# dhansmair/flamingo-mini

Hardware: AMD Instinct MI355X
Metric: images/sec (fwd+bwd) flamingo-mini bs=32 (higher is better)
Workload: dtype bf16

## Files before the change

flamingo-mini_amd/csrc/ff_api.hip:

```cpp
#include <stdarg.h>
#include <stdio.h>
#include <math.h>
#include <stdlib.h>
#include "ff_common.h"
#include "ff_internal.h"

namespace ff {

static thread_local char g_err[512] = "";
void set_error(const char* fmt, ...) {
    va_list ap;
    va_start(ap, fmt);
    vsnprintf(g_err, sizeof(g_err), fmt, ap);
    va_end(ap);
}
#ifdef FF_DEBUG
int dbg_switch(const char* name, int dflt) {
    const char* e = getenv(name);
    return e ? atoi(e) : dflt;
}
#endif
int check_launch(const char* what) {
    hipError_t e = hipGetLastError();
    if (e != hipSuccess) {
        set_error("%s: launch failed: %s", what, hipGetErrorString(e));
        return FF_ERR_LAUNCH;
    }
    return FF_OK;
}


static LnArgs ln_args(int dtype, int rows, int cols, RowMap x, RowMap y, RowMap dx) {
    LnArgs a;
    a.dtype = dtype; a.rows = rows; a.cols = cols;
    a.x_map = x; a.y_map = y; a.dx_map = dx;
    a.add_rows_per_seg = 0; a.add_div = 0; a.eps = 1e-5f; a.stats_given = 0;
    return a;
}

struct RsDims {
    int dt, Bn, T, v, D, F, q, H, dh, inner, ffi, R, depth, nte, act;
    int Mq, Mkv, Mf;
    size_t es, attn_ws;
    float scale;
    RowMap pD, pI, pF;
    RowMap lat_bcast;
    RowMap kv_media, kv_lat;
    explicit RsDims(const ff_resampler_desc& d) {
        dt = d.dtype; Bn = d.batch; T = d.n_frames; v = d.n_tokens; D = d.dim; F = T * v; q = d.num_latents;
        H = d.heads; dh = d.dim_head; inner = H * dh; ffi = d.ff_mult * D; R = F + q; depth = d.depth;
        nte = d.num_time_embeds; act = d.act; es = dtype_size(dt); scale = 1.0f / sqrtf((float)dh);
        Mq = Bn * q; Mkv = Bn * R; Mf = Bn * F; attn_ws = (size_t)Bn * H * q * 4;
        pD = plain_rows(D); pI = plain_rows(inner); pF = plain_rows(ffi);
        lat_bcast = RowMap{D, 0, q};
        kv_media = RowMap{D, (long long)R * D, F};
        kv_lat = RowMap{D, (long long)R * D, q};
    }
    LnArgs ln_latents() const { return ln_args(dt, Mq, D, pD, pD, pD); }
    LnArgs ln_media(RowMap y) const {
        LnArgs a = ln_args(dt, Mf, D, pD, y, pD);
        a.add_rows_per_seg = F; a.add_div = v;
        return a;
    }
    template <typename P> P* kv_latent_rows(P* kv) const { return (P*)((char*)kv + (size_t)F * D * es); }
};
struct RsLayerSaved {
    void *x_in, *kv_in, *Qs, *K, *V, *O, *x_mid, *xn_f, *Hpre, *Aact;
    float *mean_l, *rstd_l, *lse, *mean_f, *rstd_f;
};
constexpr int kMaxDepth = 64;
struct RsSaved {
    float *mean_m, *rstd_m, *mean_o, *rstd_o;
    void* x_last;
    RsLayerSaved L[kMaxDepth];
};
static void rs_take_layer_saved(const RsDims& s, Arena& a, RsLayerSaved& L) {
    const size_t rows_q = s.Mq, rows_kv = s.Mkv;
    L.mean_l = a.take<float>(rows_q * 4);
    L.rstd_l = a.take<float>(rows_q * 4);
    L.kv_in = a.take(rows_kv * s.D * s.es);
    L.Qs = a.take(rows_q * s.inner * s.es);
    L.K = a.take(rows_kv * s.inner * s.es);
    L.V = a.take(rows_kv * s.inner * s.es);
    L.lse = a.take<float>((size_t)s.Bn * s.H * s.q * 4);
    L.O = a.take(rows_q * s.inner * s.es);
    L.x_mid = a.take(rows_q * s.D * s.es);
    L.mean_f = a.take<float>(rows_q * 4);
    L.rstd_f = a.take<float>(rows_q * 4);
    L.xn_f = a.take(rows_q * s.D * s.es);
    L.Hpre = a.take(rows_q * s.ffi * s.es);
    L.Aact = a.take(rows_q * s.ffi * s.es);
}
static size_t rs_saved_layout(const RsDims& s, void* base, size_t cap, RsSaved& o) {
    Arena a(base, cap);
    const size_t rows_q = s.Mq;
    o.mean_m = a.take<float>((size_t)s.Mf * 4);
    o.rstd_m = a.take<float>((size_t)s.Mf * 4);
    for (int l = 0; l < s.depth; l++) {
        o.L[l].x_in = l == 0 ? nullptr : a.take(rows_q * s.D * s.es);
        rs_take_layer_saved(s, a, o.L[l]);
    }
    o.x_last = a.take(rows_q * s.D * s.es);
    o.mean_o = a.take<float>(rows_q * 4);
    o.rstd_o = a.take<float>(rows_q * 4);
    return align_up(a.used);
}

static size_t rs_ws_bytes(const RsDims& s) {
    size_t w = 0;
    auto g = [&](int M, int N, int K, int nz) { w = std::max(w, gemm_workspace_bytes(s.dt, M, N, K, nz, 0)); };
    g(s.Mq, s.inner, s.D, 1); g(s.Mkv, s.inner, s.D, 2); g(s.Mq, s.D, s.inner, 1); g(s.Mq, s.ffi, s.D, 1); g(s.Mq, s.D, s.ffi, 1);
    for (int nz = 1; nz <= 4; nz++) {
        g(s.D, s.ffi, s.Mq, nz); g(s.ffi, s.D, s.Mq, nz); g(s.D, s.inner, s.Mq, nz); g(s.inner, s.D, s.Mq, nz); g(s.inner, s.D, s.Mkv, nz);
    }
    g(s.Mkv, s.D, s.inner, 1);
    w = std::max(w, layernorm_bwd_workspace(s.Mf, s.D));
    w = std::max(w, layernorm_bwd_workspace(s.Mq, s.D));
    w = std::max(w, rows_reduce_workspace(s.Mq, s.D, s.q, 1));
    w = std::max(w, rows_reduce_workspace(s.Mf, s.D, s.F, s.v));
    return align_up(w) + align_up(s.attn_ws);
}
struct RsChain {
    void *ws, *dxn, *dO, *dkv, *dln;
    size_t ws_bytes, gws;
    float* attn_ws;
};
struct RsLayerGrads {
    void *dx_mid, *dH, *dQs, *dK, *dV;
};
static void rs_take_ws(const RsDims& s, Arena& a, RsChain& c) {
    c.ws_bytes = rs_ws_bytes(s);
    c.ws = a.take(c.ws_bytes);
    c.gws = c.ws_bytes - align_up(s.attn_ws);
    c.attn_ws = c.ws ? (float*)((char*)c.ws + c.gws) : nullptr;
}
static void rs_take_chain(const RsDims& s, Arena& a, RsChain& c) {
    c.dxn = a.take((size_t)s.Mq * s.D * s.es);
    c.dO = a.take((size_t)s.Mq * s.inner * s.es);
    c.dkv = a.take((size_t)s.Mkv * s.D * s.es);
    c.dln = a.take((size_t)s.Mq * s.D * s.es);
}
static void rs_take_layer_grads(const RsDims& s, Arena& a, RsLayerGrads& g) {
    g.dx_mid = a.take((size_t)s.Mq * s.D * s.es);
    g.dH = a.take((size_t)s.Mq * s.ffi * s.es);
    g.dQs = a.take((size_t)s.Mq * s.inner * s.es);
    g.dK = a.take((size_t)s.Mkv * s.inner * s.es);
    g.dV = a.take((size_t)s.Mkv * s.inner * s.es);
}
static void rs_take_ln_partials(const RsDims& s, Arena& a, bool deferrable, float** lnp) {
    for (int i = 0; i < 3; i++) lnp[i] = deferrable ? a.take<float>(layernorm_bwd_partial_bytes(i == 2 ? s.Mf : s.Mq, s.D)) : nullptr;
}

struct RsScratch {
    RsChain c;
    void *dx0, *dxf;
    void* dx_out[kMaxDepth];
    RsLayerGrads L[kMaxDepth];
    float* lnp[3 * kMaxDepth + 1];
};
static size_t rs_scratch_layout(const RsDims& s, void* base, size_t cap, bool bwd, RsScratch& o) {
    Arena a(base, cap);
    rs_take_ws(s, a, o.c);
    if (bwd) {
        o.dx0 = a.take((size_t)s.Mq * s.D * s.es);
        rs_take_chain(s, a, o.c);
        o.dxf = a.take((size_t)s.Mf * s.D * s.es);
        for (int l = 0; l < s.depth; l++) {
            o.dx_out[l] = a.take((size_t)s.Mq * s.D * s.es);
            rs_take_layer_grads(s, a, o.L[l]);
        }
        static const int defer_ln = dbg_switch("FF_DEFER_LN", 1);
        const bool lnd = defer_ln != 0 && layernorm_bwd_deferrable(s.dt, s.D);
        for (int l = 0; l < s.depth; l++) rs_take_ln_partials(s, a, lnd, o.lnp + 3 * l);
        o.lnp[3 * s.depth] = lnd ? a.take<float>(layernorm_bwd_partial_bytes(s.Mq, s.D)) : nullptr;
    }
    return align_up(a.used);
}

static int rs_check(const ff_resampler_desc* d) {
    FF_CHECK(d, FF_ERR_SHAPE, "resampler: null descriptor");
    FF_CHECK(d->dtype == FF_DTYPE_F32 || d->dtype == FF_DTYPE_BF16, FF_ERR_UNSUPPORTED, "resampler: dtype %d", d->dtype);
    FF_CHECK(d->batch > 0 && d->n_frames > 0 && d->n_tokens > 0 && d->dim > 0 && d->depth > 0 && d->depth <= kMaxDepth && d->heads > 0 &&
                 d->dim_head > 0 && d->num_latents > 0 && d->ff_mult > 0,
             FF_ERR_SHAPE, "resampler: bad dimensions");
    FF_CHECK(d->n_frames <= d->num_time_embeds, FF_ERR_SHAPE, "resampler: %d frames > num_time_embeds %d (perceiver_resampler.py:166)",
             d->n_frames, d->num_time_embeds);
    FF_CHECK(d->act >= FF_ACT_GELU && d->act <= FF_ACT_RELU, FF_ERR_SHAPE, "resampler: act %d", d->act);
    return FF_OK;
}

static ff_attn_desc rs_attn_desc(const RsDims& s) {
    ff_attn_desc a = {};
    a.dtype = s.dt; a.batch = s.Bn; a.heads = s.H; a.dim_head = s.dh; a.n_q = s.q; a.n_kv = s.R; a.mode = FF_ATTN_DENSE;
    const ff_strides sq = {(long long)s.q * s.inner, s.inner, s.dh}, sk = {(long long)s.R * s.inner, s.inner, s.dh};
    a.q = sq; a.o = sq; a.dq = sq; a.dout = sq;
    a.k = sk; a.v = sk; a.dk = sk; a.dv = sk;
    return a;
}

static int rs_media_stats(const RsDims& s, const void* x_f, const void* tpe, float* mean_m, float* rstd_m, hipStream_t st) {
    return layernorm_fwd(s.ln_media(s.pD), x_f, tpe, nullptr, nullptr, nullptr, mean_m, rstd_m, st);
}

static int rs_layer_forward(const RsDims& s, const void* const* p, const void* x_f, const void* tpe, float* mean_m, float* rstd_m, const void* x_in,
                            RowMap x_map, void* x_out, const RsLayerSaved& L, void* ws, size_t ws_bytes, hipStream_t st) {
    const RowMap pD = s.pD, pI = s.pI, pF = s.pF;
    void* kv_lat_base = s.kv_latent_rows(L.kv_in);
    {
        LnArgs a = s.ln_media(s.kv_media);
        a.stats_given = 1;
        FF_TRY(layernorm_fwd(a, x_f, tpe, p[0], p[1], L.kv_in, mean_m, rstd_m, st));
    }
    FF_TRY(layernorm_fwd(ln_args(s.dt, s.Mq, s.D, x_map, s.kv_lat, pD), x_in, nullptr, p[2], p[3], kv_lat_base, L.mean_l, L.rstd_l, st));
    FF_TRY(Gemm(s.dt, s.Mq, s.inner, s.D).a(0, s.kv_lat).b(0, pD).c(pI).scale(s.scale).problem(kv_lat_base, p[4], L.Qs).run(ws, ws_bytes, st));
    FF_TRY(Gemm(s.dt, s.Mkv, s.inner, s.D).a(0, pD).b(0, pD).c(pI).problem(L.kv_in, p[5], L.K).problem(L.kv_in, p[6], L.V).run(ws, ws_bytes, st));
    FF_TRY(attention_fwd(rs_attn_desc(s), L.Qs, L.K, L.V, nullptr, L.O, L.lse, st));
    FF_TRY(Gemm(s.dt, s.Mq, s.D, s.inner).a(0, pI).b(0, pI).c(pD).res_map(x_map).problem(L.O, p[7], L.x_mid, nullptr, nullptr, x_in).run(ws, ws_bytes, st));
    FF_TRY(layernorm_fwd(s.ln_latents(), L.x_mid, nullptr, p[8], p[9], L.xn_f, L.mean_f, L.rstd_f, st));
    FF_TRY(Gemm(s.dt, s.Mq, s.ffi, s.D).a(0, pD).b(0, pD).c(pF).act(s.act).problem(L.xn_f, p[10], L.Aact, L.Hpre).run(ws, ws_bytes, st));
    return Gemm(s.dt, s.Mq, s.D, s.ffi).a(0, pF).b(0, pF).c(pD).problem(L.Aact, p[11], x_out, nullptr, nullptr, L.x_mid).run(ws, ws_bytes, st);
}

static int rs_final_norm(const RsDims& s, const void* x_last, const void* gamma, const void* beta, void* out, float* mean, float* rstd, hipStream_t st) {
    return layernorm_fwd(s.ln_latents(), x_last, nullptr, gamma, beta, out, mean, rstd, st);
}

static int rs_ln_bwd(const RsChain& W, float* partial, LnPending* pending, const LnArgs& a, const void* dy, const void* x, const void* add,
                     const void* gamma, const float* mean, const float* rstd, void* dx, const void* dx_res, void* dg, void* db, hipStream_t st) {
    if (partial)
        return layernorm_bwd(a, dy, x, add, gamma, mean, rstd, dx, dx_res, dg, db, partial, layernorm_bwd_partial_bytes(a.rows, a.cols), st, nullptr, pending);
    return layernorm_bwd(a, dy, x, add, gamma, mean, rstd, dx, dx_res, dg, db, W.ws, W.gws, st);
}

static int rs_layer_backward(const RsDims& s, const void* const* p, void* const* g, const void* x_f, const void* tpe, const float* mean_m,
                             const float* rstd_m, const void* x_in, RowMap x_map, const RsLayerSaved& L, const void* dx_out, void* dx_in,
                             void* dx_f, const void* dx_f_res, const RsChain& W, const RsLayerGrads& T, float* const* lnp, LnPending* ln_sets,
                             hipStream_t st) {
    const RowMap pD = s.pD, pI = s.pI, pF = s.pF;
    FF_TRY(Gemm(s.dt, s.Mq, s.ffi, s.D).a(0, pD).b(1, pF).c(pF).act_bwd(s.act).problem(dx_out, p[11], T.dH, nullptr, L.Hpre).run(W.ws, W.gws, st));
    FF_TRY(Gemm(s.dt, s.Mq, s.D, s.ffi).a(0, pF).b(1, pD).c(pD).problem(T.dH, p[10], W.dxn).run(W.ws, W.gws, st));
    FF_TRY(rs_ln_bwd(W, lnp[0], &ln_sets[0], s.ln_latents(), W.dxn, L.x_mid, nullptr, p[8], L.mean_f, L.rstd_f, T.dx_mid, dx_out, g[8], g[9], st));
    FF_TRY(Gemm(s.dt, s.Mq, s.inner, s.D).a(0, pD).b(1, pI).c(pI).problem(T.dx_mid, p[7], W.dO).run(W.ws, W.gws, st));
    FF_TRY(attention_bwd(rs_attn_desc(s), L.Qs, L.K, L.V, nullptr, L.O, W.dO, L.lse, T.dQs, T.dK, T.dV, W.attn_ws, s.attn_ws, st));
    FF_TRY(Gemm(s.dt, s.Mkv, s.D, s.inner).a(0, pI).b(1, pD).c(pD).problem(T.dK, p[5], W.dkv).run(W.ws, W.gws, st));
    FF_TRY(Gemm(s.dt, s.Mkv, s.D, s.inner).a(0, pI).b(1, pD).c(pD).problem(T.dV, p[6], W.dkv, nullptr, nullptr, W.dkv).run(W.ws, W.gws, st));
    FF_TRY(Gemm(s.dt, s.Mq, s.D, s.inner).a(0, pI).b(1, pD).c(pD).res_map(s.kv_lat).scale(s.scale)
               .problem(T.dQs, p[4], W.dln, nullptr, nullptr, s.kv_latent_rows(W.dkv)).run(W.ws, W.gws, st));
    FF_TRY(rs_ln_bwd(W, lnp[1], &ln_sets[1], ln_args(s.dt, s.Mq, s.D, x_map, pD, pD), W.dln, x_in, nullptr, p[2], L.mean_l, L.rstd_l, dx_in, T.dx_mid, g[2],
                     g[3], st));
    return rs_ln_bwd(W, lnp[2], &ln_sets[2], s.ln_media(s.kv_media), W.dkv, x_f, tpe, p[0], mean_m, rstd_m, dx_f, dx_f_res, g[0], g[1], st);
}

static int rs_input_grads(const RsDims& s, const void* dx0, const void* dxf, void* d_latents, void* d_tpe, void* ws, size_t ws_bytes, hipStream_t st) {
    FF_TRY(rows_reduce(s.dt, s.Mq, s.D, s.pD, s.q, 1, dx0, d_latents, ws, ws_bytes, st));
    if (s.nte > s.T) FF_TRY(zero_bytes((char*)d_tpe + (size_t)s.T * s.D * s.es, (size_t)(s.nte - s.T) * s.D * s.es, st));
    return rows_reduce(s.dt, s.Mf, s.D, s.pD, s.F, s.v, dxf, d_tpe, ws, ws_bytes, st);
}

static int resampler_fwd(const ff_resampler_desc* d, const void* x_f, const void* const* P, void* out, void* saved, size_t saved_bytes,
                         void* scratch, size_t scratch_bytes, hipStream_t st) {
    FF_TRY(rs_check(d));
    FF_CHECK(x_f && P && out && saved && scratch, FF_ERR_SHAPE, "resampler_fwd: null argument");
    const RsDims s(*d);
    RsSaved S;
    RsScratch W;
    FF_CHECK(rs_saved_layout(s, saved, saved_bytes, S) <= saved_bytes, FF_ERR_WORKSPACE, "resampler_fwd: saved buffer too small");
    FF_CHECK(rs_scratch_layout(s, scratch, scratch_bytes, false, W) <= scratch_bytes, FF_ERR_WORKSPACE, "resampler_fwd: scratch too small");
    const void *latents = P[0], *tpe = P[1];
    FF_TRY(rs_media_stats(s, x_f, tpe, S.mean_m, S.rstd_m, st));
    for (int l = 0; l < s.depth; l++) {
        const void* const* p = P + FF_RESAMPLER_GLOBAL_PARAMS + FF_RESAMPLER_LAYER_PARAMS * l;
        void* x_next = l + 1 < s.depth ? S.L[l + 1].x_in : S.x_last;
        FF_TRY(rs_layer_forward(s, p, x_f, tpe, S.mean_m, S.rstd_m, l == 0 ? latents : S.L[l].x_in, l == 0 ? s.lat_bcast : s.pD, x_next, S.L[l], W.c.ws,
                                W.c.ws_bytes, st));
    }
    return rs_final_norm(s, S.x_last, P[2], P[3], out, S.mean_o, S.rstd_o, st);
}

static int resampler_bwd(const ff_resampler_desc* d, const void* x_f, const void* const* P, const void* dout, const void* saved,
                         size_t saved_bytes, void* const* G, void* dx_f, void* scratch, size_t scratch_bytes, hipStream_t st) {
    FF_TRY(rs_check(d));
    FF_CHECK(x_f && P && dout && saved && G && scratch, FF_ERR_SHAPE, "resampler_bwd: null argument");
    const RsDims s(*d);
    RsSaved S;
    RsScratch W;
    FF_CHECK(rs_saved_layout(s, (void*)saved, saved_bytes, S) <= saved_bytes, FF_ERR_WORKSPACE, "resampler_bwd: saved buffer too small");
    FF_CHECK(rs_scratch_layout(s, scratch, scratch_bytes, true, W) <= scratch_bytes, FF_ERR_WORKSPACE, "resampler_bwd: scratch too small");
    const RowMap pD = s.pD, pI = s.pI, pF = s.pF;
    const void *latents = P[0], *tpe = P[1];
    void* dxf = dx_f ? dx_f : W.dxf;
    void* const ws = W.c.ws;
    const size_t gws = W.c.gws;

    LnPending ln_sets[3 * kMaxDepth + 1];
    FF_TRY(rs_ln_bwd(W.c, W.lnp[3 * s.depth], &ln_sets[3 * s.depth], s.ln_latents(), dout, S.x_last, nullptr, P[2], S.mean_o, S.rstd_o,
                     W.dx_out[s.depth - 1], nullptr, G[2], G[3], st));
    for (int l = s.depth - 1; l >= 0; l--) {
        const void* const* p = P + FF_RESAMPLER_GLOBAL_PARAMS + FF_RESAMPLER_LAYER_PARAMS * l;
        void* const* g = G + FF_RESAMPLER_GLOBAL_PARAMS + FF_RESAMPLER_LAYER_PARAMS * l;
        void* dx_below = l == 0 ? W.dx0 : W.dx_out[l - 1];
        FF_TRY(rs_layer_backward(s, p, g, x_f, tpe, S.mean_m, S.rstd_m, l == 0 ? latents : S.L[l].x_in, l == 0 ? s.lat_bcast : pD, S.L[l], W.dx_out[l],
                                 dx_below, dxf, l == s.depth - 1 ? nullptr : dxf, W.c, W.L[l], W.lnp + 3 * l, ln_sets + 3 * l, st));
    }
    FF_TRY(layernorm_bwd_finish(s.dt, ln_sets, 3 * s.depth + 1, st));
    constexpr int kRsGroup = 4;
    for (int l0 = 0; l0 < s.depth; l0 += kRsGroup) {
        const int l1 = std::min(s.depth, l0 + kRsGroup);
        Gemm g3(s.dt, s.D, s.ffi, s.Mq), g1(s.dt, s.ffi, s.D, s.Mq), go(s.dt, s.D, s.inner, s.Mq), gq(s.dt, s.inner, s.D, s.Mq);
        g3.a(1, pD).b(1, pF).c(pF);
        g1.a(1, pF).b(1, pD).c(pD);
        go.a(1, pD).b(1, pI).c(pI);
        gq.a(1, pI).b(1, s.kv_lat).c(pD).scale(s.scale);
        for (int l = l0; l < l1; l++) {
            void* const* g = G + FF_RESAMPLER_GLOBAL_PARAMS + FF_RESAMPLER_LAYER_PARAMS * l;
            const RsLayerSaved& L = S.L[l];
            const RsLayerGrads& T = W.L[l];
            g3.problem(W.dx_out[l], L.Aact, g[11]);
            g1.problem(T.dH, L.xn_f, g[10]);
            go.problem(T.dx_mid, L.O, g[7]);
            gq.problem(T.dQs, s.kv_latent_rows(L.kv_in), g[4]);
        }
        FF_TRY(g3.run(ws, gws, st));
        FF_TRY(g1.run(ws, gws, st));
        FF_TRY(go.run(ws, gws, st));
        FF_TRY(gq.run(ws, gws, st));
    }
    {
        Gemm gkv(s.dt, s.inner, s.D, s.Mkv);
        gkv.a(1, pI).b(1, pD).c(pD);
        for (int l = 0; l < s.depth; l++) {
            void* const* g = G + FF_RESAMPLER_GLOBAL_PARAMS + FF_RESAMPLER_LAYER_PARAMS * l;
            gkv.problem(W.L[l].dK, S.L[l].kv_in, g[5]);
            gkv.problem(W.L[l].dV, S.L[l].kv_in, g[6]);
            if (gkv.P.nz == kRsGroup || l == s.depth - 1) {
                FF_TRY(gkv.run(ws, gws, st));
                gkv.P.nz = 0;
            }
        }
    }
    return rs_input_grads(s, W.dx0, dxf, G[0], G[1], ws, gws, st);
}

struct RsProSaved { float *mean_m, *rstd_m; };
static size_t rs_pro_layout(const RsDims& s, void* base, size_t cap, RsProSaved& o) {
    Arena a(base, cap);
    o.mean_m = a.take<float>((size_t)s.Mf * 4);
    o.rstd_m = a.take<float>((size_t)s.Mf * 4);
    return align_up(a.used);
}
static size_t rs_layer_saved_layout(const RsDims& s, void* base, size_t cap, RsLayerSaved& L) {
    Arena a(base, cap);
    L.x_in = nullptr;
    rs_take_layer_saved(s, a, L);
    return align_up(a.used);
}
struct RsLayerScratch {
    RsChain c;
    RsLayerGrads g;
    float* lnp[3];
};
static size_t rs_layer_scratch_layout(const RsDims& s, void* base, size_t cap, RsLayerScratch& o) {
    Arena a(base, cap);
    rs_take_ws(s, a, o.c);
    rs_take_chain(s, a, o.c);
    rs_take_layer_grads(s, a, o.g);
    rs_take_ln_partials(s, a, layernorm_bwd_deferrable(s.dt, s.D), o.lnp);
    return align_up(a.used);
}

static int rs_prologue_fwd(const ff_resampler_desc* d, const void* x_f, const void* tpe, void* pro, size_t pro_bytes, hipStream_t st) {
    FF_TRY(rs_check(d));
    FF_CHECK(x_f && tpe && pro, FF_ERR_SHAPE, "resampler_prologue_fwd: null argument");
    const RsDims s(*d);
    RsProSaved S;
    FF_CHECK(rs_pro_layout(s, pro, pro_bytes, S) <= pro_bytes, FF_ERR_WORKSPACE, "resampler_prologue_fwd: saved buffer too small");
    return rs_media_stats(s, x_f, tpe, S.mean_m, S.rstd_m, st);
}

static int rs_layer_fwd(const ff_resampler_desc* d, const void* x_f, const void* tpe, const void* pro, size_t pro_bytes, const void* x_in,
                        int x_is_latents, const void* const* p, void* x_out, void* saved, size_t saved_bytes, void* scratch, size_t scratch_bytes,
                        hipStream_t st) {
    FF_TRY(rs_check(d));
    FF_CHECK(x_f && tpe && pro && x_in && p && x_out && saved && scratch, FF_ERR_SHAPE, "resampler_layer_fwd: null argument");
    const RsDims s(*d);
    RsProSaved Pr;
    RsLayerSaved L;
    RsLayerScratch W;
    FF_CHECK(rs_pro_layout(s, (void*)pro, pro_bytes, Pr) <= pro_bytes, FF_ERR_WORKSPACE, "resampler_layer_fwd: prologue buffer too small");
    FF_CHECK(rs_layer_saved_layout(s, saved, saved_bytes, L) <= saved_bytes, FF_ERR_WORKSPACE, "resampler_layer_fwd: saved buffer too small");
    FF_CHECK(rs_layer_scratch_layout(s, scratch, scratch_bytes, W) <= scratch_bytes, FF_ERR_WORKSPACE, "resampler_layer_fwd: scratch too small");
    return rs_layer_forward(s, p, x_f, tpe, Pr.mean_m, Pr.rstd_m, x_in, x_is_latents ? s.lat_bcast : s.pD, x_out, L, W.c.ws, W.c.ws_bytes, st);
}

static int rs_layer_bwd(const ff_resampler_desc* d, const void* x_f, const void* tpe, const void* pro, size_t pro_bytes, const void* x_in,
                        int x_is_latents, const void* const* p, const void* dx_out, const void* saved, size_t saved_bytes, void* const* g,
                        void* dx_in, void* dx_f, int dx_f_accumulate, void* scratch, size_t scratch_bytes, hipStream_t st) {
    FF_TRY(rs_check(d));
    FF_CHECK(x_f && tpe && pro && x_in && p && dx_out && saved && g && dx_in && dx_f && scratch, FF_ERR_SHAPE, "resampler_layer_bwd: null argument");
    const RsDims s(*d);
    RsProSaved Pr;
    RsLayerSaved L;
    RsLayerScratch W;
    FF_CHECK(rs_pro_layout(s, (void*)pro, pro_bytes, Pr) <= pro_bytes, FF_ERR_WORKSPACE, "resampler_layer_bwd: prologue buffer too small");
    FF_CHECK(rs_layer_saved_layout(s, (void*)saved, saved_bytes, L) <= saved_bytes, FF_ERR_WORKSPACE, "resampler_layer_bwd: saved buffer too small");
    FF_CHECK(rs_layer_scratch_layout(s, scratch, scratch_bytes, W) <= scratch_bytes, FF_ERR_WORKSPACE, "resampler_layer_bwd: scratch too small");
    const RowMap pD = s.pD, pI = s.pI, pF = s.pF;
    void* const ws = W.c.ws;
    const size_t gws = W.c.gws;
    LnPending ln_sets[3];
    FF_TRY(rs_layer_backward(s, p, g, x_f, tpe, Pr.mean_m, Pr.rstd_m, x_in, x_is_latents ? s.lat_bcast : pD, L, dx_out, dx_in, dx_f,
                             dx_f_accumulate ? dx_f : nullptr, W.c, W.g, W.lnp, ln_sets, st));
    FF_TRY(layernorm_bwd_finish(s.dt, ln_sets, 3, st));
    FF_TRY(Gemm(s.dt, s.D, s.ffi, s.Mq).a(1, pD).b(1, pF).c(pF).problem(dx_out, L.Aact, g[11]).run(ws, gws, st));
    FF_TRY(Gemm(s.dt, s.ffi, s.D, s.Mq).a(1, pF).b(1, pD).c(pD).problem(W.g.dH, L.xn_f, g[10]).run(ws, gws, st));
    FF_TRY(Gemm(s.dt, s.D, s.inner, s.Mq).a(1, pD).b(1, pI).c(pI).problem(W.g.dx_mid, L.O, g[7]).run(ws, gws, st));
    FF_TRY(Gemm(s.dt, s.inner, s.D, s.Mq).a(1, pI).b(1, s.kv_lat).c(pD).scale(s.scale).problem(W.g.dQs, s.kv_latent_rows(L.kv_in), g[4]).run(ws, gws, st));
    return Gemm(s.dt, s.inner, s.D, s.Mkv).a(1, pI).b(1, pD).c(pD).problem(W.g.dK, L.kv_in, g[5]).problem(W.g.dV, L.kv_in, g[6]).run(ws, gws, st);
}

static int rs_prologue_bwd(const ff_resampler_desc* d, const void* dx0, const void* dx_f, void* d_latents, void* d_tpe, void* scratch,
                           size_t scratch_bytes, hipStream_t st) {
    FF_TRY(rs_check(d));
    FF_CHECK(dx0 && dx_f && d_latents && d_tpe && scratch, FF_ERR_SHAPE, "resampler_prologue_bwd: null argument");
    const RsDims s(*d);
    RsLayerScratch W;
    FF_CHECK(rs_layer_scratch_layout(s, scratch, scratch_bytes, W) <= scratch_bytes, FF_ERR_WORKSPACE, "resampler_prologue_bwd: scratch too small");
    return rs_input_grads(s, dx0, dx_f, d_latents, d_tpe, W.c.ws, W.c.ws_bytes, st);
}

static int rs_epilogue_fwd(const ff_resampler_desc* d, const void* x_last, const void* gamma, const void* beta, void* out, void* epi, size_t epi_bytes,
                           hipStream_t st) {
    FF_TRY(rs_check(d));
    FF_CHECK(x_last && gamma && beta && out && epi, FF_ERR_SHAPE, "resampler_epilogue_fwd: null argument");
    const RsDims s(*d);
    const size_t rows_q = s.Mq;
    FF_CHECK(epi_bytes >= 2 * align_up(rows_q * 4), FF_ERR_WORKSPACE, "resampler_epilogue_fwd: saved buffer too small");
    return rs_final_norm(s, x_last, gamma, beta, out, (float*)epi, (float*)((char*)epi + align_up(rows_q * 4)), st);
}
static int rs_epilogue_bwd(const ff_resampler_desc* d, const void* dout, const void* x_last, const void* gamma, const void* epi, size_t epi_bytes,
                           void* dx_last, void* dgamma, void* dbeta, void* scratch, size_t scratch_bytes, hipStream_t st) {
    FF_TRY(rs_check(d));
    FF_CHECK(dout && x_last && gamma && epi && dx_last && dgamma && dbeta && scratch, FF_ERR_SHAPE, "resampler_epilogue_bwd: null argument");
    const RsDims s(*d);
    const size_t rows_q = s.Mq;
    FF_CHECK(epi_bytes >= 2 * align_up(rows_q * 4), FF_ERR_WORKSPACE, "resampler_epilogue_bwd: saved buffer too small");
    RsLayerScratch W;
    FF_CHECK(rs_layer_scratch_layout(s, scratch, scratch_bytes, W) <= scratch_bytes, FF_ERR_WORKSPACE, "resampler_epilogue_bwd: scratch too small");
    const float* mean = (const float*)epi;
    const float* rstd = (const float*)((const char*)epi + align_up(rows_q * 4));
    return layernorm_bwd(s.ln_latents(), dout, x_last, nullptr, gamma, mean, rstd, dx_last, nullptr, dgamma, dbeta, W.c.ws, W.c.ws_bytes, st);
}

struct XaDims {
    int dt, b, L, d, dv, Nm, nv, Nk, H, dh, inner, ffi, act;
    size_t es;
    float scale;
    bool ext_kv;
    explicit XaDims(const ff_xattn_desc& x) {
        ext_kv = x.cached_k.sr != 0;
        dt = x.dtype; b = x.batch; L = x.n_tokens; d = x.dim; dv = x.dim_visual; Nm = x.n_media; nv = x.n_visual; Nk = Nm * nv;
        H = x.heads; dh = x.dim_head; inner = H * dh; ffi = x.ff_mult * d; act = x.act; es = dtype_size(dt);
        scale = 1.0f / sqrtf((float)dh);
    }
};
struct XaSaved {
    float *mean_a, *rstd_a, *lse, *mean_f, *rstd_f;
    void *yn, *Qs, *KV, *O, *attn_out, *y1, *xn_f, *Hpre, *Aact, *ffw_out;
    size_t kv_offset;
};
static size_t xa_saved_layout(const XaDims& s, void* base, size_t cap, XaSaved& o) {
    Arena a(base, cap);
    const size_t M = (size_t)s.b * s.L;
    o.KV = s.ext_kv ? nullptr : a.take((size_t)s.b * s.Nk * 2 * s.inner * s.es);
    o.kv_offset = 0;
    o.mean_a = a.take<float>(M * 4);
    o.rstd_a = a.take<float>(M * 4);
    o.yn = a.take(M * s.d * s.es);
    o.Qs = a.take(M * s.inner * s.es);
    o.lse = a.take<float>((size_t)s.b * s.H * s.L * 4);
    o.O = a.take(M * s.inner * s.es);
    o.attn_out = a.take(M * s.d * s.es);
    o.y1 = a.take(M * s.d * s.es);
    o.mean_f = a.take<float>(M * 4);
    o.rstd_f = a.take<float>(M * 4);
    o.xn_f = a.take(M * s.d * s.es);
    o.Hpre = a.take(M * s.ffi * s.es);
    o.Aact = a.take(M * s.ffi * s.es);
    o.ffw_out = a.take(M * s.d * s.es);
    return align_up(a.used);
}
struct XaScratch {
    void *dy1, *dH, *dxn, *dO, *dQs, *dKV, *dyn, *ws;
    size_t ws_bytes;
    float* lnx;
};
struct XaStash {
    void *dy1, *dH, *dQs;
    float *lnp_f = nullptr, *lnp_a = nullptr;
};
static bool xa_ln_deferrable(const XaDims& s) {
    static const int on = dbg_switch("FF_DEFER_LN", 1);
    return on != 0 && layernorm_bwd_deferrable(s.dt, s.d);
}
static size_t xa_stash_layout(const XaDims& s, void* base, size_t cap, XaStash& o) {
    Arena a(base, cap);
    const size_t M = (size_t)s.b * s.L;
    o.dy1 = a.take(M * s.d * s.es);
    o.dH = a.take(M * s.ffi * s.es);
    o.dQs = a.take(M * s.inner * s.es);
    if (xa_ln_deferrable(s)) {
        o.lnp_f = a.take<float>(layernorm_bwd_partial_bytes((int)M, s.d));
        o.lnp_a = a.take<float>(layernorm_bwd_partial_bytes((int)M, s.d));
    }
    return align_up(a.used);
}
static size_t xa_ws_bytes(const XaDims& s) {
    const int M = s.b * s.L, Mk = s.b * s.Nk;
    size_t w = 0;
    auto g = [&](int m, int n, int k) { w = std::max(w, gemm_workspace_bytes(s.dt, m, n, k, 1, 0)); };
    g(M, s.inner, s.d); g(Mk, 2 * s.inner, s.dv); g(M, s.d, s.inner); g(M, s.ffi, s.d); g(M, s.d, s.ffi);
    g(s.d, s.ffi, M); g(s.ffi, s.d, M); g(s.d, s.inner, M); g(s.inner, s.d, M); g(2 * s.inner, s.dv, Mk); g(Mk, s.dv, 2 * s.inner);
    w = std::max(w, layernorm_bwd_workspace(M, s.d));
    w = std::max(w, gate_grad_workspace(M, s.d));
    if (decode_ffw_supported(s.dt, M, s.d, s.ffi)) w = std::max(w, decode_ffw_workspace_bytes(s.d, s.ffi));
    return align_up(w) + align_up((size_t)s.b * s.H * s.L * 4);
}
static size_t xa_scratch_layout(const XaDims& s, void* base, size_t cap, bool bwd, XaScratch& o) {
    Arena a(base, cap);
    const size_t M = (size_t)s.b * s.L;
    o.ws_bytes = xa_ws_bytes(s);
    o.ws = a.take(o.ws_bytes);
    o.lnx = a.take<float>(xa_ln3_part_bytes(s.b, s.H));
    if (bwd) {
        o.dy1 = a.take(M * s.d * s.es);
        o.dH = a.take(M * s.ffi * s.es);
        o.dxn = a.take(M * s.d * s.es);
        o.dO = a.take(M * s.inner * s.es);
        o.dQs = a.take(M * s.inner * s.es);
        o.dKV = s.ext_kv ? nullptr : a.take((size_t)s.b * s.Nk * 2 * s.inner * s.es);
        o.dyn = a.take(M * s.d * s.es);
    }
    return align_up(a.used);
}
static int xa_check(const ff_xattn_desc* d) {
    FF_CHECK(d, FF_ERR_SHAPE, "xattn: null descriptor");
    FF_CHECK(d->dtype == FF_DTYPE_F32 || d->dtype == FF_DTYPE_BF16, FF_ERR_UNSUPPORTED, "xattn: dtype %d", d->dtype);
    FF_CHECK(d->batch > 0 && d->n_tokens > 0 && d->dim > 0 && d->dim_visual > 0 && d->n_media > 0 && d->n_visual > 0 && d->heads > 0 &&
                 d->dim_head > 0 && d->ff_mult > 0,
             FF_ERR_SHAPE, "xattn: bad dimensions");
    FF_CHECK(d->act >= FF_ACT_GELU && d->act <= FF_ACT_RELU, FF_ERR_SHAPE, "xattn: act %d", d->act);
    return FF_OK;
}
static ff_attn_desc xa_attn_desc(const ff_xattn_desc& x, const XaDims& s, bool cached) {
    ff_attn_desc a = {};
    a.dtype = s.dt; a.batch = s.b; a.heads = s.H; a.dim_head = s.dh; a.n_q = s.L; a.n_kv = s.Nk;
    a.mode = FF_ATTN_MEDIA; a.n_visual = s.nv; a.tt_stride = x.tt_stride; a.tt_offset = x.tt_offset;
    const ff_strides sq = {(long long)s.L * s.inner, s.inner, s.dh};
    const ff_strides sk = {(long long)s.Nk * 2 * s.inner, 2LL * s.inner, s.dh};
    a.q = sq; a.o = sq; a.dq = sq; a.dout = sq;
    a.k = cached ? x.cached_k : sk;
    a.v = cached ? x.cached_v : sk;
    a.dk = sk; a.dv = sk;
    return a;
}

static bool xa_fused_enabled() {
    static const int v = dbg_switch("FF_XATTN_FUSED", 1);
    return v != 0;
}
static bool xa_ln3_enabled() {
    static const int v = dbg_switch("FF_XATTN_LN3", 1);
    return v != 0;
}
static XaFusedArgs xa_fused_args(const ff_xattn_desc& x, const XaDims& s, bool ext_kv) {
    XaFusedArgs a = {};
    a.batch = s.b; a.heads = s.H; a.n_q = s.L; a.n_kv = s.Nk; a.n_visual = s.nv; a.tt_stride = x.tt_stride; a.tt_offset = x.tt_offset;
    a.dim = s.d; a.inner = s.inner; a.scale = s.scale; a.eps = 1e-5f;
    static const int xcd_split = dbg_switch("FF_XATTN_XCD_SPLIT", 0);
    a.xcd_split = xcd_split;
    const ff_strides sk = {(long long)s.Nk * 2 * s.inner, 2LL * s.inner, s.dh};
    a.k = ext_kv ? x.cached_k : sk;
    a.v = ext_kv ? x.cached_v : sk;
    a.dk = sk; a.dv = sk;
    return a;
}

static bool xa_ln3_in_bwd(const ff_xattn_desc& x, const XaDims& s) {
    if (!xa_ln3_enabled() || !xa_fused_enabled() || !xa_fused_supported(s.dt, s.dh, s.d, s.inner) || x.sync == nullptr) return false;
    const XaFusedArgs fa = xa_fused_args(x, s, s.ext_kv);
    const int M = s.b * s.L;
    return xa_out_fusable(fa, s.dt, s.dh) && s.b <= layernorm_bwd_partial_blocks(M) && (size_t)s.b * (2 * (size_t)s.d + 2) * sizeof(float) <= layernorm_bwd_workspace(M, s.d);
}
static int xattn_fwd(const ff_xattn_desc* d, const void* y, const void* vf, const int* tt, const void* const* P, const void* ck,
                     const void* cv, void* y_out, void* saved, size_t saved_bytes, void* scratch, size_t scratch_bytes, hipStream_t st) {
    FF_TRY(xa_check(d));
    const bool cached = ck != nullptr;
    FF_CHECK(y && tt && P && y_out && saved && scratch && (cached ? cv != nullptr : vf != nullptr), FF_ERR_SHAPE, "xattn_fwd: null argument");
    const XaDims s(*d);
    FF_CHECK(s.ext_kv == cached, FF_ERR_SHAPE, "xattn_fwd: external K / V need their strides in the descriptor (cached_k / cached_v) and vice versa");
    XaSaved S;
    XaScratch W;
    FF_CHECK(xa_saved_layout(s, saved, saved_bytes, S) <= saved_bytes, FF_ERR_WORKSPACE, "xattn_fwd: saved buffer too small");
    FF_CHECK(xa_scratch_layout(s, scratch, scratch_bytes, false, W) <= scratch_bytes, FF_ERR_WORKSPACE, "xattn_fwd: scratch too small");
    const int M = s.b * s.L, Mk = s.b * s.Nk;
    const RowMap pd = plain_rows(s.d), pI = plain_rows(s.inner), pF = plain_rows(s.ffi), pV = plain_rows(s.dv), pKV = plain_rows(2 * s.inner);
    const void *Kp, *Vp;
    if (!cached) {
        FF_TRY(Gemm(s.dt, Mk, 2 * s.inner, s.dv).a(0, pV).b(0, pV).c(pKV).problem(vf, P[5], S.KV).run(W.ws, W.ws_bytes, st));
        Kp = S.KV;
        Vp = (const char*)S.KV + (size_t)s.inner * s.es;
    } else {
        Kp = ck; Vp = cv;
    }
    bool out_fused = false, ln_fused = false;
    if (xa_fused_enabled() && xa_fused_supported(s.dt, s.dh, s.d, s.inner)) {
        const XaFusedArgs fa = xa_fused_args(*d, s, cached);
        XaOutArgs oa = {(const bf16*)P[6], (const bf16*)P[0], (bf16*)S.y1, (bf16*)S.attn_out, (unsigned*)d->sync};
        out_fused = d->sync != nullptr && xa_out_fusable(fa, s.dt, s.dh) && !decode_ffw_supported(s.dt, M, s.d, s.ffi);
        if (out_fused && xa_ln3_enabled()) {
            oa.ln_g = (const bf16*)P[7]; oa.ln_b = (const bf16*)P[8]; oa.ln_out = (bf16*)S.xn_f; oa.ln_mean = S.mean_f; oa.ln_rstd = S.rstd_f;
            oa.ln_part = W.lnx;
            ln_fused = true;
        }
        FF_TRY(xa_qattn_fwd(fa, s.dt, s.dh, y, P[2], P[3], P[4], Kp, Vp, tt, S.yn, S.Qs, S.O, S.mean_a, S.rstd_a, S.lse, st, out_fused ? &oa : nullptr));
    } else {
        FF_TRY(layernorm_fwd(ln_args(s.dt, M, s.d, pd, pd, pd), y, nullptr, P[2], P[3], S.yn, S.mean_a, S.rstd_a, st));
        FF_TRY(Gemm(s.dt, M, s.inner, s.d).a(0, pd).b(0, pd).c(pI).scale(s.scale).problem(S.yn, P[4], S.Qs).run(W.ws, W.ws_bytes, st));
        FF_TRY(attention_fwd(xa_attn_desc(*d, s, cached), S.Qs, Kp, Vp, tt, S.O, S.lse, st));
    }
    if (!out_fused) FF_TRY(Gemm(s.dt, M, s.d, s.inner).a(0, pI).b(0, pI).c(pd).problem(S.O, P[6], S.y1, S.attn_out, nullptr, y, P[0]).run(W.ws, W.ws_bytes, st));
    if (decode_ffw_supported(s.dt, M, s.d, s.ffi))
        return decode_ffw(M, s.d, s.ffi, s.act, 1e-5f, S.y1, P[7], P[8], P[9], P[10], P[1], S.xn_f, S.mean_f, S.rstd_f, S.Hpre, S.Aact, S.ffw_out, y_out,
                          W.ws, W.ws_bytes, st);
    if (!ln_fused) FF_TRY(layernorm_fwd(ln_args(s.dt, M, s.d, pd, pd, pd), S.y1, nullptr, P[7], P[8], S.xn_f, S.mean_f, S.rstd_f, st));
    FF_TRY(Gemm(s.dt, M, s.ffi, s.d).a(0, pd).b(0, pd).c(pF).act(s.act).problem(S.xn_f, P[9], S.Aact, S.Hpre).run(W.ws, W.ws_bytes, st));
    return Gemm(s.dt, M, s.d, s.ffi).a(0, pF).b(0, pF).c(pd).problem(S.Aact, P[10], y_out, S.ffw_out, nullptr, S.y1, P[1]).run(W.ws, W.ws_bytes, st);
}

static int xattn_bwd(const ff_xattn_desc* d, const void* y, const void* vf, const int* tt, const void* const* P, const void* dy2,
                     const void* saved, size_t saved_bytes, void* const* G, void* dy, void* dvf, void* scratch, size_t scratch_bytes,
                     hipStream_t st, const void* ext_k = nullptr, const void* ext_v = nullptr, void* dkv_out = nullptr,
                     void* stash = nullptr, size_t stash_bytes = 0) {
    FF_TRY(xa_check(d));
    const bool hoisted = ext_k != nullptr;
    FF_CHECK(y && tt && P && dy2 && saved && G && dy && scratch && (hoisted ? (ext_v && dkv_out) : vf != nullptr), FF_ERR_SHAPE,
             "xattn_bwd: null argument");
    const XaDims s(*d);
    FF_CHECK(s.ext_kv == hoisted, FF_ERR_SHAPE, "xattn_bwd: external K / V need their strides in the descriptor (cached_k / cached_v) and vice versa");
    XaSaved S;
    XaScratch W;
    FF_CHECK(xa_saved_layout(s, (void*)saved, saved_bytes, S) <= saved_bytes, FF_ERR_WORKSPACE, "xattn_bwd: saved buffer too small");
    FF_CHECK(xa_scratch_layout(s, scratch, scratch_bytes, true, W) <= scratch_bytes, FF_ERR_WORKSPACE, "xattn_bwd: scratch too small");
    XaStash T{W.dy1, W.dH, W.dQs};
    const bool defer = stash != nullptr;
    if (defer) FF_CHECK(xa_stash_layout(s, stash, stash_bytes, T) <= stash_bytes, FF_ERR_WORKSPACE, "xattn_bwd: stash too small");
    const bool defer_ln = defer && xa_ln_deferrable(s);
    if (defer_ln)
        FF_CHECK(((uintptr_t)y | (uintptr_t)dy | (uintptr_t)dy2 | (uintptr_t)P[2] | (uintptr_t)P[7]) % 16 == 0, FF_ERR_SHAPE,
                 "xattn_bwd (deferred weight gradients): y, d y_out, d y and the LayerNorm weights must be 16-byte aligned");
    LnPending pend_f, pend_a;
    const int M = s.b * s.L, Mk = s.b * s.Nk;
    const RowMap pd = plain_rows(s.d), pI = plain_rows(s.inner), pF = plain_rows(s.ffi), pV = plain_rows(s.dv), pKV = plain_rows(2 * s.inner);
    const size_t attn_ws_bytes = align_up((size_t)s.b * s.H * s.L * 4);
    const size_t gws = W.ws_bytes - attn_ws_bytes;
    float* attn_ws = (float*)((char*)W.ws + gws);

    if (!defer) FF_TRY(Gemm(s.dt, s.d, s.ffi, M).a(1, pd).b(1, pF).c(pF).problem(dy2, S.Aact, G[10], nullptr, nullptr, nullptr, P[1]).run(W.ws, gws, st));
    FF_TRY(Gemm(s.dt, M, s.ffi, s.d).a(0, pd).b(1, pF).c(pF).act_bwd(s.act).problem(dy2, P[10], T.dH, nullptr, S.Hpre, nullptr, P[1]).run(W.ws, gws, st));
    if (!defer) FF_TRY(Gemm(s.dt, s.ffi, s.d, M).a(1, pF).b(1, pd).c(pd).problem(T.dH, S.xn_f, G[9]).run(W.ws, gws, st));
    static const int fold_reduce = dbg_switch("FF_FOLD_SPLITK_LN", 1);
    int dxn_splits = 1;
    FF_TRY(Gemm(s.dt, M, s.d, s.ffi).a(0, pF).b(1, pd).c(pd).problem(T.dH, P[9], W.dxn).run(W.ws, gws, st, defer_ln && fold_reduce ? &dxn_splits : nullptr));
    {
        LnDots dots;
        dots.a = S.ffw_out; dots.alpha_a = P[1]; dots.out_a = G[1];
        dots.b = S.attn_out; dots.alpha_b = P[0]; dots.out_b = G[0];
        if (defer_ln) {
            LnArgs la = ln_args(s.dt, M, s.d, pd, pd, pd);
            if (dxn_splits > 1) { la.dy_splits = dxn_splits; la.dy_slab = (long long)M * s.d; }
            FF_TRY(layernorm_bwd(la, dxn_splits > 1 ? W.ws : W.dxn, S.y1, nullptr, P[7], S.mean_f, S.rstd_f, T.dy1, dy2, G[7], G[8], T.lnp_f,
                                 layernorm_bwd_partial_bytes(M, s.d), st, &dots, &pend_f));
            FF_CHECK(pend_f.partial, FF_ERR_SHAPE, "xattn_bwd: the one-pass LayerNorm backward did not apply in the deferred mode");
        } else FF_TRY(layernorm_bwd(ln_args(s.dt, M, s.d, pd, pd, pd), W.dxn, S.y1, nullptr, P[7], S.mean_f, S.rstd_f, T.dy1, dy2, G[7], G[8], W.ws, gws, st, &dots));
    }
    if (!defer) FF_TRY(Gemm(s.dt, s.d, s.inner, M).a(1, pd).b(1, pI).c(pI).problem(T.dy1, S.O, G[6], nullptr, nullptr, nullptr, P[0]).run(W.ws, gws, st));
    char* dK = hoisted ? (char*)dkv_out : (char*)W.dKV;
    char* dV = dK + (size_t)s.inner * s.es;
    const void* Kp = hoisted ? ext_k : S.KV;
    const void* Vp = hoisted ? ext_v : (const void*)((const char*)S.KV + (size_t)s.inner * s.es);
    bool dyn_fused = false, lnb_fused = false;
    float* lnb_partial = nullptr;
    if (xa_fused_enabled() && xa_fused_supported(s.dt, s.dh, s.d, s.inner)) {
        int single = 0;
        const XaFusedArgs fa = xa_fused_args(*d, s, hoisted);
        XaOutArgs oa = {(const bf16*)P[4], nullptr, (bf16*)W.dyn, nullptr, (unsigned*)d->sync};
        dyn_fused = d->sync != nullptr && xa_out_fusable(fa, s.dt, s.dh);
        if (dyn_fused && xa_ln3_in_bwd(*d, s)) {
            lnb_fused = true;
            lnb_partial = defer_ln ? T.lnp_a : (float*)W.ws;
            oa.out = nullptr;
            oa.ln_g = (const bf16*)P[2]; oa.ln_x = (const bf16*)y; oa.ln_res = (const bf16*)T.dy1; oa.ln_out = (bf16*)dy;
            oa.ln_mean = S.mean_a; oa.ln_rstd = S.rstd_a; oa.ln_part = W.lnx; oa.ln_wpart = lnb_partial;
        }
        FF_TRY(xa_dattn_bwd(fa, s.dt, s.dh, T.dy1, P[6], P[0], S.Qs, Kp, Vp, tt, S.O, S.lse, W.dO, T.dQs, dK, dV, attn_ws, &single, st,
                            dyn_fused ? &oa : nullptr));
        if (!single) FF_TRY(attention_bwd_dkv(xa_attn_desc(*d, s, hoisted), S.Qs, Kp, Vp, tt, W.dO, S.lse, attn_ws, dK, dV, st));
        if (lnb_fused && !defer_ln) {
            LnPending q;
            q.partial = lnb_partial; q.nblk = s.b; q.cols = s.d; q.dgamma = G[2]; q.dbeta = G[3];
            FF_TRY(layernorm_bwd_finish(s.dt, &q, 1, st));
        }
    } else {
        FF_TRY(Gemm(s.dt, M, s.inner, s.d).a(0, pd).b(1, pI).c(pI).problem(T.dy1, P[6], W.dO, nullptr, nullptr, nullptr, P[0]).run(W.ws, gws, st));
        FF_TRY(attention_bwd(xa_attn_desc(*d, s, hoisted), S.Qs, Kp, Vp, tt, S.O, W.dO, S.lse, T.dQs, dK, dV, attn_ws, (size_t)s.b * s.H * s.L * 4, st));
    }
    if (!defer) FF_TRY(Gemm(s.dt, s.inner, s.d, M).a(1, pI).b(1, pd).c(pd).scale(s.scale).problem(T.dQs, S.yn, G[4]).run(W.ws, gws, st));
    if (!hoisted) {
        FF_TRY(Gemm(s.dt, 2 * s.inner, s.dv, Mk).a(1, pKV).b(1, pV).c(pV).problem(W.dKV, vf, G[5]).run(W.ws, gws, st));
        if (dvf) FF_TRY(Gemm(s.dt, Mk, s.dv, 2 * s.inner).a(0, pKV).b(1, pV).c(pV).problem(W.dKV, P[5], dvf).run(W.ws, gws, st));
    }
    if (!dyn_fused) FF_TRY(Gemm(s.dt, M, s.d, s.inner).a(0, pI).b(1, pd).c(pd).scale(s.scale).problem(T.dQs, P[4], W.dyn).run(W.ws, gws, st));
    if (lnb_fused) return FF_OK;
    if (defer_ln) {
        FF_TRY(layernorm_bwd(ln_args(s.dt, M, s.d, pd, pd, pd), W.dyn, y, nullptr, P[2], S.mean_a, S.rstd_a, dy, T.dy1, G[2], G[3], T.lnp_a,
                             layernorm_bwd_partial_bytes(M, s.d), st, nullptr, &pend_a));
        FF_CHECK(pend_a.partial, FF_ERR_SHAPE, "xattn_bwd: the one-pass LayerNorm backward did not apply in the deferred mode");
        return FF_OK;
    }
    return layernorm_bwd(ln_args(s.dt, M, s.d, pd, pd, pd), W.dyn, y, nullptr, P[2], S.mean_a, S.rstd_a, dy, T.dy1, G[2], G[3], W.ws, gws, st);
}

static size_t xa_wgrad_ws_bytes(const XaDims& s) {
    const int M = s.b * s.L;
    size_t w = 0;
    for (int nz = 1; nz <= kGemmMaxZ; nz++)
        w = std::max({w, gemm_workspace_bytes(s.dt, s.d, s.ffi, M, nz, 0), gemm_workspace_bytes(s.dt, s.ffi, s.d, M, nz, 0),
                      gemm_workspace_bytes(s.dt, s.d, s.inner, M, nz, 0), gemm_workspace_bytes(s.dt, s.inner, s.d, M, nz, 0)});
    return align_up(w);
}
static int xattn_wgrad_grouped(const ff_xattn_desc* d, int n, const void* const* dy2, const void* const* saved, size_t saved_bytes,
                               const void* const* stash, size_t stash_bytes, const void* const* params, void* const* grads, void* ws,
                               size_t ws_bytes, hipStream_t st) {
    FF_TRY(xa_check(d));
    FF_CHECK(n >= 1 && n <= kGemmMaxZ && dy2 && saved && stash && params && grads, FF_ERR_SHAPE, "xattn_wgrad_grouped: 1..%d blocks per call", kGemmMaxZ);
    const XaDims s(*d);
    FF_CHECK(ws_bytes >= xa_wgrad_ws_bytes(s) && (ws || !xa_wgrad_ws_bytes(s)), FF_ERR_WORKSPACE, "xattn_wgrad_grouped: workspace too small");
    const int M = s.b * s.L;
    const RowMap pd = plain_rows(s.d), pI = plain_rows(s.inner), pF = plain_rows(s.ffi);
    LnPending ln_sets[2 * kGemmMaxZ];
    const bool finish_ln = xa_ln_deferrable(s);
    const int ln_blocks = layernorm_bwd_partial_blocks(M);
    Gemm g3(s.dt, s.d, s.ffi, M), g1(s.dt, s.ffi, s.d, M), go(s.dt, s.d, s.inner, M), gq(s.dt, s.inner, s.d, M);
    g3.a(1, pd).b(1, pF).c(pF);
    g1.a(1, pF).b(1, pd).c(pd);
    go.a(1, pd).b(1, pI).c(pI);
    gq.a(1, pI).b(1, pd).c(pd).scale(s.scale);
    for (int i = 0; i < n; i++) {
        XaSaved S;
        XaStash T;
        FF_CHECK(dy2[i] && saved[i] && stash[i], FF_ERR_SHAPE, "xattn_wgrad_grouped: null buffer of block %d", i);
        FF_CHECK(xa_saved_layout(s, (void*)saved[i], saved_bytes, S) <= saved_bytes, FF_ERR_WORKSPACE, "xattn_wgrad_grouped: saved buffer too small");
        FF_CHECK(xa_stash_layout(s, (void*)stash[i], stash_bytes, T) <= stash_bytes, FF_ERR_WORKSPACE, "xattn_wgrad_grouped: stash too small");
        const void* const* P = params + (size_t)i * FF_XATTN_PARAMS;
        void* const* G = grads + (size_t)i * FF_XATTN_PARAMS;
        FF_CHECK(G[10] && G[9] && G[6] && G[4] && P[0] && P[1], FF_ERR_SHAPE, "xattn_wgrad_grouped: null parameter / gradient of block %d", i);
        g3.problem(dy2[i], S.Aact, G[10], nullptr, nullptr, nullptr, P[1]);
        g1.problem(T.dH, S.xn_f, G[9]);
        go.problem(T.dy1, S.O, G[6], nullptr, nullptr, nullptr, P[0]);
        gq.problem(T.dQs, S.yn, G[4]);
        if (finish_ln) {
            FF_CHECK(G[0] && G[1] && G[2] && G[3] && G[7] && G[8], FF_ERR_SHAPE, "xattn_wgrad_grouped: null LayerNorm / gate gradient of block %d", i);
            LnPending& f = ln_sets[2 * i];
            f.partial = T.lnp_f; f.nblk = ln_blocks; f.cols = s.d; f.dgamma = G[7]; f.dbeta = G[8];
            f.alpha_a = P[1]; f.out_a = G[1]; f.alpha_b = P[0]; f.out_b = G[0];
            LnPending& q = ln_sets[2 * i + 1];
            q.partial = T.lnp_a; q.nblk = xa_ln3_in_bwd(*d, s) ? s.b : ln_blocks; q.cols = s.d; q.dgamma = G[2]; q.dbeta = G[3];
        }
    }
    if (finish_ln) FF_TRY(layernorm_bwd_finish(s.dt, ln_sets, 2 * n, st));
    FF_TRY(g3.run(ws, ws_bytes, st));
    FF_TRY(g1.run(ws, ws_bytes, st));
    FF_TRY(go.run(ws, ws_bytes, st));
    return gq.run(ws, ws_bytes, st);
}

static int kvp_check(const ff_kvproj_desc* d) {
    FF_CHECK(d, FF_ERR_SHAPE, "kv_project: null descriptor");
    FF_CHECK(d->dtype == FF_DTYPE_F32 || d->dtype == FF_DTYPE_BF16, FF_ERR_UNSUPPORTED, "kv_project: dtype %d", d->dtype);
    FF_CHECK(d->n_layers > 0 && d->rows > 0 && d->dim_visual > 0 && d->kv_dim > 0 && (long long)d->rows * d->dim_visual < (1LL << 31), FF_ERR_SHAPE,
             "kv_project: bad dimensions");
    return FF_OK;
}
static size_t kvp_gemm_ws(const ff_kvproj_desc* d) {
    size_t w = 0;
    for (int z = 1; z <= kKvProjGroup; z++)
        w = std::max({w, gemm_workspace_bytes(d->dtype, d->rows, d->kv_dim, d->dim_visual, z, 0),
                      gemm_workspace_bytes(d->dtype, d->kv_dim, d->dim_visual, d->rows, z, 0),
                      gemm_workspace_bytes(d->dtype, d->rows, d->dim_visual, d->kv_dim, z, 0)});
    return align_up(w);
}
static size_t kvp_ws_bytes(const ff_kvproj_desc* d, bool with_dvf) {
    const size_t es = d->dtype == FF_DTYPE_BF16 ? 2 : 4;
    size_t w = kvp_gemm_ws(d);
    if (with_dvf)
        w += align_up((size_t)d->n_layers * d->rows * d->dim_visual * es) +
             align_up(rows_reduce_workspace(d->n_layers, d->rows * d->dim_visual, d->n_layers, d->n_layers));
    return w;
}
static int kv_project_fwd(const ff_kvproj_desc* d, const void* vf, const void* const* w_kv, void* const* kv_out, void* ws, size_t ws_bytes,
                          hipStream_t st) {
    FF_TRY(kvp_check(d));
    FF_CHECK(vf && w_kv && kv_out && ws && ws_bytes >= kvp_gemm_ws(d), FF_ERR_WORKSPACE, "kv_project_fwd: null argument or workspace too small");
    const RowMap pV = plain_rows(d->dim_visual), pKV = plain_rows(d->kv_dim);
    for (int l0 = 0; l0 < d->n_layers; l0 += kKvProjGroup) {
        Gemm g(d->dtype, d->rows, d->kv_dim, d->dim_visual);
        g.a(0, pV).b(0, pV).c(pKV);
        for (int l = l0; l < std::min(d->n_layers, l0 + kKvProjGroup); l++) g.problem(vf, w_kv[l], kv_out[l]);
        FF_TRY(g.run(ws, ws_bytes, st));
    }
    return FF_OK;
}
static int kv_project_bwd(const ff_kvproj_desc* d, const void* vf, const void* const* w_kv, const void* const* dkv, void* const* dw_kv,
                          void* dvf, void* ws, size_t ws_bytes, hipStream_t st) {
    FF_TRY(kvp_check(d));
    FF_CHECK(vf && w_kv && dkv && dw_kv && ws && ws_bytes >= kvp_ws_bytes(d, dvf != nullptr), FF_ERR_WORKSPACE,
             "kv_project_bwd: null argument or workspace too small");
    const size_t es = d->dtype == FF_DTYPE_BF16 ? 2 : 4, gws = kvp_gemm_ws(d);
    const RowMap pV = plain_rows(d->dim_visual), pKV = plain_rows(d->kv_dim);
    char* terms = (char*)ws + gws;
    const size_t term_bytes = (size_t)d->rows * d->dim_visual * es;
    for (int l0 = 0; l0 < d->n_layers; l0 += kKvProjGroup) {
        const int l1 = std::min(d->n_layers, l0 + kKvProjGroup);
        Gemm gw(d->dtype, d->kv_dim, d->dim_visual, d->rows);
        gw.a(1, pKV).b(1, pV).c(pV);
        for (int l = l0; l < l1; l++) gw.problem(dkv[l], vf, dw_kv[l]);
        FF_TRY(gw.run(ws, gws, st));
        if (dvf) {
            Gemm gx(d->dtype, d->rows, d->dim_visual, d->kv_dim);
            gx.a(0, pKV).b(1, pV).c(pV);
            for (int l = l0; l < l1; l++) gx.problem(dkv[l], w_kv[l], terms + (size_t)l * term_bytes);
            FF_TRY(gx.run(ws, gws, st));
        }
    }
    if (dvf) {
        const int cols = d->rows * d->dim_visual;
        FF_TRY(rows_reduce(d->dtype, d->n_layers, cols, plain_rows(cols), d->n_layers, d->n_layers, terms, dvf,
                           terms + align_up((size_t)d->n_layers * term_bytes), rows_reduce_workspace(d->n_layers, cols, d->n_layers, d->n_layers), st));
    }
    return FF_OK;
}

}

extern "C" int ff_version(void) { return 6; }
extern "C" const char* ff_arch(void) { return "gfx950"; }
extern "C" const char* ff_last_error(void) { return ff::g_err; }

extern "C" size_t ff_resampler_saved_bytes(const ff_resampler_desc* d) {
    if (ff::rs_check(d) != FF_OK) return 0;
    ff::RsSaved S;
    return ff::rs_saved_layout(ff::RsDims(*d), nullptr, 0, S);
}
extern "C" size_t ff_resampler_scratch_bytes(const ff_resampler_desc* d) {
    if (ff::rs_check(d) != FF_OK) return 0;
    ff::RsScratch W;
    return ff::rs_scratch_layout(ff::RsDims(*d), nullptr, 0, true, W);
}
extern "C" int ff_resampler_fwd(const ff_resampler_desc* d, const void* x_f, const void* const* params, void* out, void* saved,
                                size_t saved_bytes, void* scratch, size_t scratch_bytes, ff_stream_t stream) {
    return ff::resampler_fwd(d, x_f, params, out, saved, saved_bytes, scratch, scratch_bytes, (hipStream_t)stream);
}
extern "C" int ff_resampler_bwd(const ff_resampler_desc* d, const void* x_f, const void* const* params, const void* dout,
                                const void* saved, size_t saved_bytes, void* const* grads, void* dx_f, void* scratch,
                                size_t scratch_bytes, ff_stream_t stream) {
    return ff::resampler_bwd(d, x_f, params, dout, saved, saved_bytes, grads, dx_f, scratch, scratch_bytes, (hipStream_t)stream);
}

extern "C" size_t ff_resampler_prologue_saved_bytes(const ff_resampler_desc* d) {
    if (ff::rs_check(d) != FF_OK) return 0;
    ff::RsProSaved S;
    return ff::rs_pro_layout(ff::RsDims(*d), nullptr, 0, S);
}
extern "C" size_t ff_resampler_layer_saved_bytes(const ff_resampler_desc* d) {
    if (ff::rs_check(d) != FF_OK) return 0;
    ff::RsLayerSaved L;
    return ff::rs_layer_saved_layout(ff::RsDims(*d), nullptr, 0, L);
}
extern "C" size_t ff_resampler_layer_scratch_bytes(const ff_resampler_desc* d) {
    if (ff::rs_check(d) != FF_OK) return 0;
    ff::RsLayerScratch W;
    return ff::rs_layer_scratch_layout(ff::RsDims(*d), nullptr, 0, W);
}
extern "C" size_t ff_resampler_epilogue_saved_bytes(const ff_resampler_desc* d) {
    if (ff::rs_check(d) != FF_OK) return 0;
    return 2 * ff::align_up((size_t)d->batch * d->num_latents * 4);
}
extern "C" int ff_resampler_prologue_fwd(const ff_resampler_desc* d, const void* x_f, const void* time_pos_emb, void* saved_pro, size_t saved_pro_bytes,
                                         hipStream_t stream) {
    return ff::rs_prologue_fwd(d, x_f, time_pos_emb, saved_pro, saved_pro_bytes, stream);
}
extern "C" int ff_resampler_layer_fwd(const ff_resampler_desc* d, const void* x_f, const void* time_pos_emb, const void* saved_pro, size_t saved_pro_bytes,
                                      const void* x_in, int x_in_is_latents, const void* const* layer_params, void* x_out, void* saved, size_t saved_bytes,
                                      void* scratch, size_t scratch_bytes, hipStream_t stream) {
    return ff::rs_layer_fwd(d, x_f, time_pos_emb, saved_pro, saved_pro_bytes, x_in, x_in_is_latents, layer_params, x_out, saved, saved_bytes, scratch,
                            scratch_bytes, stream);
}
extern "C" int ff_resampler_layer_bwd(const ff_resampler_desc* d, const void* x_f, const void* time_pos_emb, const void* saved_pro, size_t saved_pro_bytes,
                                      const void* x_in, int x_in_is_latents, const void* const* layer_params, const void* dx_out, const void* saved,
                                      size_t saved_bytes, void* const* layer_grads, void* dx_in, void* dx_f, int dx_f_accumulate, void* scratch,
                                      size_t scratch_bytes, hipStream_t stream) {
    return ff::rs_layer_bwd(d, x_f, time_pos_emb, saved_pro, saved_pro_bytes, x_in, x_in_is_latents, layer_params, dx_out, saved, saved_bytes, layer_grads,
                            dx_in, dx_f, dx_f_accumulate, scratch, scratch_bytes, stream);
}
extern "C" int ff_resampler_prologue_bwd(const ff_resampler_desc* d, const void* dx0, const void* dx_f, void* d_latents, void* d_time_pos_emb, void* scratch,
                                         size_t scratch_bytes, hipStream_t stream) {
    return ff::rs_prologue_bwd(d, dx0, dx_f, d_latents, d_time_pos_emb, scratch, scratch_bytes, stream);
}
extern "C" int ff_resampler_epilogue_fwd(const ff_resampler_desc* d, const void* x_last, const void* norm_weight, const void* norm_bias, void* out,
                                         void* saved_epi, size_t saved_epi_bytes, hipStream_t stream) {
    return ff::rs_epilogue_fwd(d, x_last, norm_weight, norm_bias, out, saved_epi, saved_epi_bytes, stream);
}
extern "C" int ff_resampler_epilogue_bwd(const ff_resampler_desc* d, const void* dout, const void* x_last, const void* norm_weight, const void* saved_epi,
                                         size_t saved_epi_bytes, void* dx_last, void* d_norm_weight, void* d_norm_bias, void* scratch, size_t scratch_bytes,
                                         hipStream_t stream) {
    return ff::rs_epilogue_bwd(d, dout, x_last, norm_weight, saved_epi, saved_epi_bytes, dx_last, d_norm_weight, d_norm_bias, scratch, scratch_bytes, stream);
}

extern "C" size_t ff_xattn_sync_bytes(void) { return (size_t)(4 * FF_XATTN_SYNC_SLOTS + 64) * sizeof(unsigned); }
extern "C" int ff_xattn_sync_status(const void* sync, hipStream_t stream) {
    FF_CHECK(sync, FF_ERR_SHAPE, "ff_xattn_sync_status: null buffer");
    unsigned flag = 0;
    hipError_t e = hipMemcpyAsync(&flag, (const unsigned*)sync + 2 * FF_XATTN_SYNC_SLOTS, sizeof(flag), hipMemcpyDeviceToHost, stream);
    if (e == hipSuccess) e = hipStreamSynchronize(stream);
    FF_CHECK(e == hipSuccess, FF_ERR_LAUNCH, "ff_xattn_sync_status: %s", hipGetErrorString(e));
    return flag ? 1 : 0;
}
extern "C" size_t ff_xattn_saved_bytes(const ff_xattn_desc* d) {
    if (ff::xa_check(d) != FF_OK) return 0;
    ff::XaSaved S;
    return ff::xa_saved_layout(ff::XaDims(*d), nullptr, 0, S);
}
extern "C" size_t ff_xattn_scratch_bytes(const ff_xattn_desc* d) {
    if (ff::xa_check(d) != FF_OK) return 0;
    ff::XaScratch W;
    return ff::xa_scratch_layout(ff::XaDims(*d), nullptr, 0, true, W);
}
extern "C" size_t ff_xattn_kv_offset(const ff_xattn_desc* d) {
    (void)d;
    return 0;
}
extern "C" int ff_xattn_block_fwd(const ff_xattn_desc* d, const void* y, const void* visual_features, const int* text_time,
                                  const void* const* params, const void* cached_k, const void* cached_v, void* y_out, void* saved,
                                  size_t saved_bytes, void* scratch, size_t scratch_bytes, ff_stream_t stream) {
    return ff::xattn_fwd(d, y, visual_features, text_time, params, cached_k, cached_v, y_out, saved, saved_bytes, scratch, scratch_bytes,
                         (hipStream_t)stream);
}
extern "C" int ff_xattn_block_bwd(const ff_xattn_desc* d, const void* y, const void* visual_features, const int* text_time,
                                  const void* const* params, const void* dy_out, const void* saved, size_t saved_bytes, void* const* grads,
                                  void* dy, void* dvisual_features, void* scratch, size_t scratch_bytes, ff_stream_t stream) {
    return ff::xattn_bwd(d, y, visual_features, text_time, params, dy_out, saved, saved_bytes, grads, dy, dvisual_features, scratch,
                         scratch_bytes, (hipStream_t)stream);
}

extern "C" int ff_xattn_block_bwd_kv(const ff_xattn_desc* d, const void* y, const void* k, const void* v, const int* text_time,
                                     const void* const* params, const void* dy_out, const void* saved, size_t saved_bytes,
                                     void* const* grads, void* dy, void* dkv, void* scratch, size_t scratch_bytes, ff_stream_t stream) {
    using namespace ff;
    FF_CHECK(k && v && dkv, FF_ERR_SHAPE, "ff_xattn_block_bwd_kv: null K / V / dKV");
    return xattn_bwd(d, y, nullptr, text_time, params, dy_out, saved, saved_bytes, grads, dy, nullptr, scratch, scratch_bytes,
                     (hipStream_t)stream, k, v, dkv);
}
extern "C" size_t ff_xattn_wgrad_stash_bytes(const ff_xattn_desc* d) {
    if (ff::xa_check(d) != FF_OK) return 0;
    ff::XaStash T;
    return ff::xa_stash_layout(ff::XaDims(*d), nullptr, 0, T);
}
extern "C" size_t ff_xattn_wgrad_workspace_bytes(const ff_xattn_desc* d) {
    if (ff::xa_check(d) != FF_OK) return 0;
    return ff::xa_wgrad_ws_bytes(ff::XaDims(*d));
}
extern "C" int ff_xattn_block_bwd_kv_data(const ff_xattn_desc* d, const void* y, const void* k, const void* v, const int* text_time,
                                          const void* const* params, const void* dy_out, const void* saved, size_t saved_bytes,
                                          void* const* grads, void* dy, void* dkv, void* stash, size_t stash_bytes, void* scratch,
                                          size_t scratch_bytes, ff_stream_t stream) {
    using namespace ff;
    FF_CHECK(k && v && dkv && stash, FF_ERR_SHAPE, "ff_xattn_block_bwd_kv_data: null K / V / dKV / stash");
    return xattn_bwd(d, y, nullptr, text_time, params, dy_out, saved, saved_bytes, grads, dy, nullptr, scratch, scratch_bytes,
                     (hipStream_t)stream, k, v, dkv, stash, stash_bytes);
}
extern "C" int ff_xattn_wgrad_grouped(const ff_xattn_desc* d, int n_blocks, const void* const* dy_out, const void* const* saved,
                                      size_t saved_bytes, const void* const* stash, size_t stash_bytes, const void* const* params,
                                      void* const* grads, void* workspace, size_t workspace_bytes, ff_stream_t stream) {
    return ff::xattn_wgrad_grouped(d, n_blocks, dy_out, saved, saved_bytes, stash, stash_bytes, params, grads, workspace, workspace_bytes,
                                   (hipStream_t)stream);
}
extern "C" size_t ff_kv_project_workspace_bytes(const ff_kvproj_desc* d, int with_dvf) {
    if (ff::kvp_check(d) != FF_OK) return 0;
    return ff::kvp_ws_bytes(d, with_dvf != 0);
}
extern "C" int ff_kv_project_fwd(const ff_kvproj_desc* d, const void* visual_features, const void* const* w_kv, void* const* kv_out,
                                 void* workspace, size_t workspace_bytes, ff_stream_t stream) {
    return ff::kv_project_fwd(d, visual_features, w_kv, kv_out, workspace, workspace_bytes, (hipStream_t)stream);
}
extern "C" int ff_kv_project_bwd(const ff_kvproj_desc* d, const void* visual_features, const void* const* w_kv, const void* const* dkv,
                                 void* const* dw_kv, void* dvisual_features, void* workspace, size_t workspace_bytes, ff_stream_t stream) {
    return ff::kv_project_bwd(d, visual_features, w_kv, dkv, dw_kv, dvisual_features, workspace, workspace_bytes, (hipStream_t)stream);
}
```

flamingo-mini_amd/csrc/ff_internal.h:

```cpp
#pragma once
#include <algorithm>
#include "ff_common.h"

namespace ff {

constexpr int kGemmMaxZ = 12;
constexpr int kKvProjGroup = 4;
struct GemmProblem {
    const void* A;
    const void* B;
    void* C;
    void* aux_out;
    const void* aux_in;
    const void* residual;
    const void* gate;
};
struct GemmParams {
    int M, N, K;
    int a_layout, b_layout;
    RowMap a_map, b_map, c_map, r_map;
    float scale;
    int act, act_bwd;
    int split_k, k_per_split;
    int tile;
    int force_tile, force_stages;
    int xcd_ms, xcd_ns;
    float* partial;
    int a_vec_ok, b_vec_ok;
    int c_vec8;
    int nz;
    GemmProblem p[kGemmMaxZ];
};
int gemm_pick_split(int dtype, int M, int N, int K, int nz);
size_t gemm_workspace_bytes(int dtype, int M, int N, int K, int nz, int split_k);
int gemm_launch(GemmParams P, int dtype, void* workspace, size_t ws_bytes, hipStream_t st, int* leave_partial = nullptr);

struct Gemm {
    GemmParams P;
    int dtype;
    Gemm(int dtype_, int M, int N, int K) : dtype(dtype_) {
        P = GemmParams{};
        P.M = M; P.N = N; P.K = K;
        P.scale = 1.f; P.act = FF_ACT_NONE; P.act_bwd = FF_ACT_NONE; P.split_k = 0; P.nz = 0;
        P.a_map = plain_rows(K); P.b_map = plain_rows(K); P.c_map = plain_rows(N); P.r_map = P.c_map;
    }
    Gemm& a(int layout, RowMap m) { P.a_layout = layout; P.a_map = m; return *this; }
    Gemm& b(int layout, RowMap m) { P.b_layout = layout; P.b_map = m; return *this; }
    Gemm& c(RowMap m) { P.c_map = m; P.r_map = m; return *this; }
    Gemm& res_map(RowMap m) { P.r_map = m; return *this; }
    Gemm& scale(float s) { P.scale = s; return *this; }
    Gemm& act(int a) { P.act = a; return *this; }
    Gemm& act_bwd(int a) { P.act_bwd = a; return *this; }
    Gemm& problem(const void* A, const void* B, void* C, void* aux_out = nullptr, const void* aux_in = nullptr,
                  const void* residual = nullptr, const void* gate = nullptr) {
        P.p[P.nz++] = GemmProblem{A, B, C, aux_out, aux_in, residual, gate};
        return *this;
    }
    size_t workspace() const { return gemm_workspace_bytes(dtype, P.M, P.N, P.K, std::max(P.nz, 1), P.split_k); }
    int run(void* ws, size_t ws_bytes, hipStream_t st, int* leave_partial = nullptr) const { return gemm_launch(P, dtype, ws, ws_bytes, st, leave_partial); }
};

int profile_begin(int dtype, int tile, int a_layout, int b_layout, int M, int N, int K, int nz, int split_k, hipStream_t st);
void profile_end(int i, hipStream_t st);

struct LnArgs {
    int dtype;
    int rows, cols;
    RowMap x_map, y_map, dx_map;
    int add_rows_per_seg, add_div;
    float eps;
    int stats_given;
    int dy_splits = 0;
    long long dy_slab = 0;
};
int layernorm_fwd(const LnArgs& a, const void* x, const void* add, const void* gamma, const void* beta, void* y,
                  float* mean, float* rstd, hipStream_t st);
size_t layernorm_bwd_workspace(int rows, int cols);
struct LnDots {
    const void* a = nullptr; const void* alpha_a = nullptr; void* out_a = nullptr;
    const void* b = nullptr; const void* alpha_b = nullptr; void* out_b = nullptr;
};
struct LnPending {
    const float* partial = nullptr;
    int nblk = 0, cols = 0;
    void *dgamma = nullptr, *dbeta = nullptr;
    const void* alpha_a = nullptr; void* out_a = nullptr;
    const void* alpha_b = nullptr; void* out_b = nullptr;
};
constexpr int kLnFinishMax = 8;
bool layernorm_bwd_deferrable(int dtype, int cols);
size_t layernorm_bwd_partial_bytes(int rows, int cols);
int layernorm_bwd_partial_blocks(int rows);
int layernorm_bwd(const LnArgs& a, const void* dy, const void* x, const void* add, const void* gamma, const float* mean,
                  const float* rstd, void* dx, const void* dx_residual, void* dgamma, void* dbeta, void* ws,
                  size_t ws_bytes, hipStream_t st, const LnDots* dots = nullptr, LnPending* pending = nullptr);
int layernorm_bwd_finish(int dtype, const LnPending* sets, int n, hipStream_t st);
size_t rows_reduce_workspace(int rows, int cols, int rows_per_batch, int rows_per_group);
int zero_bytes(void* p, size_t bytes, hipStream_t st);
int rows_reduce(int dtype, int rows, int cols, RowMap x_map, int rows_per_batch, int rows_per_group, const void* x,
                void* out, void* ws, size_t ws_bytes, hipStream_t st);
size_t gate_grad_workspace(int rows, int cols);
int gate_grad(int dtype, int rows, int cols, const void* a, const void* b, const void* alpha, void* dalpha, void* ws,
              size_t ws_bytes, hipStream_t st);
int text_time(int batch, int n_tokens, const void* ml, int elem_bytes, int* out, hipStream_t st);

size_t attention_bwd_workspace(const ff_attn_desc& d);
int attention_fwd(const ff_attn_desc& d, const void* Q, const void* K, const void* V, const int* tt, void* O, float* lse,
                  hipStream_t st);
int attention_bwd(const ff_attn_desc& d, const void* Q, const void* K, const void* V, const int* tt, const void* O,
                  const void* dO, const float* lse, void* dQ, void* dK, void* dV, void* ws, size_t ws_bytes,
                  hipStream_t st);

int attention_bwd_dkv(const ff_attn_desc& d, const void* Q, const void* K, const void* V, const int* tt, const void* dO, const float* lse,
                      const float* Dsum, void* dK, void* dV, hipStream_t st);

struct XaFusedArgs {
    int batch, heads, n_q, n_kv, n_visual, tt_stride, tt_offset;
    int dim, inner;
    float scale, eps;
    int xcd_split;
    ff_strides k, v, dk, dv;
};
struct XaOutArgs {
    const bf16* W;
    const bf16* gate;
    bf16* out;
    bf16* aux;
    unsigned* sync;
    const bf16* ln_g;
    const bf16* ln_b;
    bf16* ln_out;
    float* ln_mean;
    float* ln_rstd;
    const bf16* ln_x;
    const bf16* ln_res;
    float* ln_part;
    float* ln_wpart;
};
size_t xa_ln3_part_bytes(int batch, int heads);
bool xa_out_fusable(const XaFusedArgs& a, int dtype, int dim_head);
bool xa_fused_supported(int dtype, int dim_head, int dim, int inner);
int xa_qattn_fwd(const XaFusedArgs& a, int dtype, int dim_head, const void* y, const void* gamma, const void* beta, const void* Wq, const void* K,
                 const void* V, const int* tt, void* yn, void* Qs, void* O, float* mean, float* rstd, float* lse, hipStream_t st,
                 const XaOutArgs* out = nullptr);
int xa_dattn_bwd(const XaFusedArgs& a, int dtype, int dim_head, const void* dy1, const void* Wo, const void* gate, const void* Qs, const void* K,
                 const void* V, const int* tt, const void* O, const float* lse, void* dO, void* dQ, void* dK, void* dV, float* Dsum,
                 int* single_tile, hipStream_t st, const XaOutArgs* out = nullptr);

bool decode_ffw_supported(int dtype, int M, int d, int ffi);
size_t decode_ffw_workspace_bytes(int d, int ffi);
int decode_ffw(int M, int d, int ffi, int act, float eps, const void* y1, const void* gamma, const void* beta, const void* W1, const void* W3,
               const void* alpha, void* xn, float* mean, float* rstd, void* Hpre, void* Aact, void* ffw_out, void* y_out, void* ws, size_t ws_bytes,
               hipStream_t st);

struct Arena {
    unsigned char* base;
    size_t cap, used;
    Arena(void* p, size_t c) : base((unsigned char*)p), cap(c), used(0) {}
    template <typename T = void> T* take(size_t bytes) {
        size_t at = align_up(used);
        used = at + bytes;
        return (T*)(base ? base + at : nullptr);
    }
    bool ok() const { return used <= cap; }
};

}
```

flamingo-mini_amd/csrc/ff_rowwise.hip:

```cpp
#include "ff_common.h"
#include "ff_internal.h"

namespace ff {

#ifdef FF_XA_TIMELINE
__device__ unsigned long long g_ln_timeline[4096 * 8];
#define FF_LTL(i) do { if (threadIdx.x == 0 && blockIdx.x < 4096) g_ln_timeline[blockIdx.x * 8 + (i)] = __builtin_amdgcn_s_memrealtime(); } while (0)
#else
#define FF_LTL(i) do { } while (0)
#endif

template <typename T, int VEC> FF_DEV void ld(const T* p, float (&o)[VEC]) {
    if constexpr (VEC == 1) o[0] = to_f32(p[0]);
    else Vec<T>::load(p, o);
}
template <typename T, int VEC> FF_DEV void st(T* p, const float (&o)[VEC]) {
    if constexpr (VEC == 1) p[0] = from_f32<T>(o[0]);
    else Vec<T>::store(p, o);
}

template <typename T, int VEC>
__global__ __launch_bounds__(256) void ln_fwd_kernel(const LnArgs a_in, const T* __restrict__ x, const T* __restrict__ add,
                                                     const T* __restrict__ gamma, const T* __restrict__ beta, T* __restrict__ y,
                                                     float* __restrict__ mean, float* __restrict__ rstd) {
    const LnArgs a = fetch_args(a_in);
    pin_args(x, add, gamma, beta, y, mean, rstd);
    const int lane = threadIdx.x & 63;
    const int row = blockIdx.x * 4 + (threadIdx.x >> 6);
    if (row >= a.rows) return;
    const T* xr = x + a.x_map.off(row);
    const T* ar = nullptr;
    if (add) ar = add + (long long)((row % a.add_rows_per_seg) / a.add_div) * a.cols;
    const int nchunk = a.cols / VEC;
    float mu, rs;
    if (nchunk <= 4 * 64 && VEC > 1) {
        float v[4][VEC];
#pragma unroll
        for (int u = 0; u < 4; u++) {
            const int c = lane + 64 * u;
            if (c < nchunk) {
                ld<T, VEC>(xr + c * VEC, v[u]);
                if (ar) {
                    float t[VEC];
                    ld<T, VEC>(ar + c * VEC, t);
#pragma unroll
                    for (int i = 0; i < VEC; i++) v[u][i] += t[i];
                }
            }
        }
        if (a.stats_given) {
            mu = mean[row];
            rs = rstd[row];
        } else {
            float s = 0.f;
#pragma unroll
            for (int u = 0; u < 4; u++)
                if (lane + 64 * u < nchunk)
#pragma unroll
                    for (int i = 0; i < VEC; i++) s += v[u][i];
            mu = wave_sum(s) / (float)a.cols;
            float q = 0.f;
#pragma unroll
            for (int u = 0; u < 4; u++)
                if (lane + 64 * u < nchunk)
#pragma unroll
                    for (int i = 0; i < VEC; i++) q += (v[u][i] - mu) * (v[u][i] - mu);
            rs = rsqrtf(wave_sum(q) / (float)a.cols + a.eps);
            if (lane == 0 && mean) {
                mean[row] = mu;
                rstd[row] = rs;
            }
        }
        if (!y) return;
        T* yr = y + a.y_map.off(row);
#pragma unroll
        for (int u = 0; u < 4; u++) {
            const int c = lane + 64 * u;
            if (c < nchunk) {
                float g[VEC], b[VEC], o[VEC];
                ld<T, VEC>(gamma + c * VEC, g);
                ld<T, VEC>(beta + c * VEC, b);
#pragma unroll
                for (int i = 0; i < VEC; i++) o[i] = (v[u][i] - mu) * rs * g[i] + b[i];
                st<T, VEC>(yr + c * VEC, o);
            }
        }
        return;
    }
    if (a.stats_given) {
        mu = mean[row];
        rs = rstd[row];
    } else {
        float s = 0.f;
        for (int c = lane; c < nchunk; c += 64) {
            float v[VEC];
            ld<T, VEC>(xr + c * VEC, v);
            if (ar) {
                float t[VEC];
                ld<T, VEC>(ar + c * VEC, t);
#pragma unroll
                for (int i = 0; i < VEC; i++) v[i] += t[i];
            }
#pragma unroll
            for (int i = 0; i < VEC; i++) s += v[i];
        }
        mu = wave_sum(s) / (float)a.cols;
        float q = 0.f;
        for (int c = lane; c < nchunk; c += 64) {
            float v[VEC];
            ld<T, VEC>(xr + c * VEC, v);
            if (ar) {
                float t[VEC];
                ld<T, VEC>(ar + c * VEC, t);
#pragma unroll
                for (int i = 0; i < VEC; i++) v[i] += t[i];
            }
#pragma unroll
            for (int i = 0; i < VEC; i++) q += (v[i] - mu) * (v[i] - mu);
        }
        rs = rsqrtf(wave_sum(q) / (float)a.cols + a.eps);
        if (lane == 0 && mean) {
            mean[row] = mu;
            rstd[row] = rs;
        }
    }
    if (!y) return;
    T* yr = y + a.y_map.off(row);
    for (int c = lane; c < nchunk; c += 64) {
        float v[VEC], g[VEC], b[VEC];
        ld<T, VEC>(xr + c * VEC, v);
        if (ar) {
            float t[VEC];
            ld<T, VEC>(ar + c * VEC, t);
#pragma unroll
            for (int i = 0; i < VEC; i++) v[i] += t[i];
        }
        ld<T, VEC>(gamma + c * VEC, g);
        ld<T, VEC>(beta + c * VEC, b);
#pragma unroll
        for (int i = 0; i < VEC; i++) v[i] = (v[i] - mu) * rs * g[i] + b[i];
        st<T, VEC>(yr + c * VEC, v);
    }
}

template <typename T, int VEC>
__global__ __launch_bounds__(256) void ln_bwd_dx_kernel(const LnArgs a_in, const T* __restrict__ dy, const T* __restrict__ x,
                                                        const T* __restrict__ add, const T* __restrict__ gamma,
                                                        const float* __restrict__ mean, const float* __restrict__ rstd, T* dx,
                                                        const T* dx_res) {
    const LnArgs a = fetch_args(a_in);
    pin_args(dy, x, add, gamma, mean, rstd, dx, dx_res);
    const int lane = threadIdx.x & 63;
    const int row = blockIdx.x * 4 + (threadIdx.x >> 6);
    if (row >= a.rows) return;
    const T* xr = x + a.x_map.off(row);
    const T* dyr = dy + a.y_map.off(row);
    const T* ar = nullptr;
    if (add) ar = add + (long long)((row % a.add_rows_per_seg) / a.add_div) * a.cols;
    const float mu = mean[row], rs = rstd[row];
    const int nchunk = a.cols / VEC;
    float s1 = 0.f, s2 = 0.f;
    for (int c = lane; c < nchunk; c += 64) {
        float v[VEC], d[VEC], g[VEC];
        ld<T, VEC>(xr + c * VEC, v);
        if (ar) {
            float t[VEC];
            ld<T, VEC>(ar + c * VEC, t);
#pragma unroll
            for (int i = 0; i < VEC; i++) v[i] += t[i];
        }
        ld<T, VEC>(dyr + c * VEC, d);
        ld<T, VEC>(gamma + c * VEC, g);
#pragma unroll
        for (int i = 0; i < VEC; i++) {
            const float dyh = d[i] * g[i];
            s1 += dyh;
            s2 += dyh * (v[i] - mu) * rs;
        }
    }
    const float m1 = wave_sum(s1) / (float)a.cols, m2 = wave_sum(s2) / (float)a.cols;
    const long long doff = a.dx_map.off(row);
    for (int c = lane; c < nchunk; c += 64) {
        float v[VEC], d[VEC], g[VEC], o[VEC];
        ld<T, VEC>(xr + c * VEC, v);
        if (ar) {
            float t[VEC];
            ld<T, VEC>(ar + c * VEC, t);
#pragma unroll
            for (int i = 0; i < VEC; i++) v[i] += t[i];
        }
        ld<T, VEC>(dyr + c * VEC, d);
        ld<T, VEC>(gamma + c * VEC, g);
#pragma unroll
        for (int i = 0; i < VEC; i++) o[i] = rs * (d[i] * g[i] - m1 - (v[i] - mu) * rs * m2);
        if (dx_res) {
            float q[VEC];
            ld<T, VEC>(dx_res + doff + c * VEC, q);
#pragma unroll
            for (int i = 0; i < VEC; i++) o[i] += q[i];
        }
        st<T, VEC>(dx + doff + c * VEC, o);
    }
}


template <typename T, int VEC, int NCH>
__global__ __launch_bounds__(256) void ln_bwd_fused_kernel(const LnArgs a_in, const T* __restrict__ dy, const T* __restrict__ x,
                                                           const T* __restrict__ add, const T* __restrict__ gamma,
                                                           const float* __restrict__ mean, const float* __restrict__ rstd, T* dx,
                                                           const T* dx_res, const T* __restrict__ dot_a, const T* __restrict__ dot_b,
                                                           float* __restrict__ partial, int rows_per_block) {
    FF_LTL(0);
    const LnArgs a = fetch_args(a_in);
    pin_args(dy, x, add, gamma, mean, rstd, dx, dx_res, dot_a, dot_b, partial, rows_per_block);
    extern __shared__ __attribute__((aligned(16))) float sacc[];
    FF_LTL(1);
    __shared__ float red[4];
    const int lane = threadIdx.x & 63, w = threadIdx.x >> 6;
    const int nchunk = a.cols / VEC;
    float accg[NCH][VEC], accb[NCH][VEC];
#pragma unroll
    for (int i = 0; i < NCH; i++)
#pragma unroll
        for (int e = 0; e < VEC; e++) accg[i][e] = accb[i][e] = 0.f;
    float da = 0.f, db = 0.f;
    const int row_end = min(a.rows, (int)(blockIdx.x + 1) * rows_per_block);
    auto load_dy = [&](int row, const T* dyr, int c, float (&d)[VEC]) {
        if (a.dy_splits > 0) {
            const float* pp = (const float*)dy + (long long)row * a.cols + c * VEC;
#pragma unroll
            for (int e = 0; e < VEC; e++) d[e] = 0.f;
            for (int sp = 0; sp < a.dy_splits; sp++) {
#pragma unroll
                for (int e = 0; e < VEC; e += 4) {
                    const f32x4 q = *(const f32x4*)(pp + (long long)sp * a.dy_slab + e);
                    d[e] += q[0]; d[e + 1] += q[1]; d[e + 2] += q[2]; d[e + 3] += q[3];
                }
            }
        } else ld<T, VEC>(dyr + c * VEC, d);
    };
    for (int row = blockIdx.x * rows_per_block + w; row < row_end; row += 4) {
        const T* xr = x + a.x_map.off(row);
        const T* dyr = a.dy_splits > 0 ? dy : dy + a.y_map.off(row);
        const T* ar = add ? add + (long long)((row % a.add_rows_per_seg) / a.add_div) * a.cols : nullptr;
        const float mu = mean[row], rs = rstd[row];
        float s1 = 0.f, s2 = 0.f;
        constexpr bool KEEP = NCH <= 4;
        constexpr bool HOIST = KEEP && VEC > 1;
        float xk[KEEP ? NCH : 1][VEC], dk[KEEP ? NCH : 1][VEC];
        uint4 rq[HOIST ? NCH : 1], ra[HOIST ? NCH : 1], rb[HOIST ? NCH : 1];
        const long long doff = a.dx_map.off(row);
#pragma unroll
        for (int i = 0; i < NCH; i++) {
            const int c = lane + 64 * i;
            if (c < nchunk) {
                float v[VEC], d[VEC], g[VEC];
                ld<T, VEC>(xr + c * VEC, v);
                if (ar) {
                    float t[VEC];
                    ld<T, VEC>(ar + c * VEC, t);
#pragma unroll
                    for (int e = 0; e < VEC; e++) v[e] += t[e];
                }
                load_dy(row, dyr, c, d);
                ld<T, VEC>(gamma + c * VEC, g);
                if constexpr (HOIST) {
                    if (dx_res) rq[i] = *(const uint4*)(dx_res + doff + c * VEC);
                    if (dot_a) ra[i] = *(const uint4*)(dot_a + doff + c * VEC);
                    if (dot_b) rb[i] = *(const uint4*)(dot_b + doff + c * VEC);
                }
#pragma unroll
                for (int e = 0; e < VEC; e++) {
                    const float dyh = d[e] * g[e], xh = (v[e] - mu) * rs;
                    s1 += dyh;
                    s2 += dyh * xh;
                    if (KEEP) { xk[i][e] = xh; dk[i][e] = d[e]; }
                }
            }
        }
        const float m1 = wave_sum(s1) / (float)a.cols, m2 = wave_sum(s2) / (float)a.cols;
        auto unpack = [](const uint4& r, float (&o)[VEC]) {
            if constexpr (VEC > 1) {
                typedef typename Vec<T>::raw raw_t;
                const raw_t x = __builtin_bit_cast(raw_t, r);
#pragma unroll
                for (int e = 0; e < VEC; e++) o[e] = to_f32(x[e]);
            }
        };
#pragma unroll
        for (int i = 0; i < NCH; i++) {
            const int c = lane + 64 * i;
            if (c < nchunk) {
                float xh[VEC], d[VEC], g[VEC], o[VEC];
                if (KEEP) {
#pragma unroll
                    for (int e = 0; e < VEC; e++) { xh[e] = xk[i][e]; d[e] = dk[i][e]; }
                } else {
                    float v[VEC];
                    ld<T, VEC>(xr + c * VEC, v);
                    if (ar) {
                        float t[VEC];
                        ld<T, VEC>(ar + c * VEC, t);
#pragma unroll
                        for (int e = 0; e < VEC; e++) v[e] += t[e];
                    }
                    load_dy(row, dyr, c, d);
#pragma unroll
                    for (int e = 0; e < VEC; e++) xh[e] = (v[e] - mu) * rs;
                }
                ld<T, VEC>(gamma + c * VEC, g);
#pragma unroll
                for (int e = 0; e < VEC; e++) {
                    o[e] = rs * (d[e] * g[e] - m1 - xh[e] * m2);
                    accg[i][e] += d[e] * xh[e];
                    accb[i][e] += d[e];
                }
                if (dx_res) {
                    float q[VEC];
                    if constexpr (HOIST) unpack(rq[i], q);
                    else ld<T, VEC>(dx_res + doff + c * VEC, q);
                    if (dot_a) {
                        float u[VEC];
                        if constexpr (HOIST) unpack(ra[i], u);
                        else ld<T, VEC>(dot_a + doff + c * VEC, u);
#pragma unroll
                        for (int e = 0; e < VEC; e++) da += q[e] * u[e];
                    }
#pragma unroll
                    for (int e = 0; e < VEC; e++) o[e] += q[e];
                }
                if (dx) {
                    float r[VEC];
#pragma unroll
                    for (int e = 0; e < VEC; e++) r[e] = to_f32(from_f32<T>(o[e]));
                    if (dot_b) {
                        float u[VEC];
                        if constexpr (HOIST) unpack(rb[i], u);
                        else ld<T, VEC>(dot_b + doff + c * VEC, u);
#pragma unroll
                        for (int e = 0; e < VEC; e++) db += r[e] * u[e];
                    }
                    st<T, VEC>(dx + doff + c * VEC, o);
                }
            }
        }
    }
    FF_LTL(2);
    {
        float* mine = sacc + (size_t)w * 2 * a.cols;
#pragma unroll
        for (int i = 0; i < NCH; i++) {
            const int c = lane + 64 * i;
            if (c < nchunk) {
#pragma unroll
                for (int e = 0; e < VEC; e += 4) {
                    *(f32x4*)(mine + c * VEC + e) = f32x4{accg[i][e], accg[i][e + 1], accg[i][e + 2], accg[i][e + 3]};
                    *(f32x4*)(mine + a.cols + c * VEC + e) = f32x4{accb[i][e], accb[i][e + 1], accb[i][e + 2], accb[i][e + 3]};
                }
            }
        }
    }
    __syncthreads();
    FF_LTL(3);
    const long long P = 2LL * a.cols + 2;
    float* out = partial + (long long)blockIdx.x * P;
    for (int i = threadIdx.x * 4; i < 2 * a.cols; i += 256 * 4) {
        const f32x4 s0 = *(const f32x4*)(sacc + i), s1 = *(const f32x4*)(sacc + 2 * a.cols + i);
        const f32x4 s2 = *(const f32x4*)(sacc + 4 * a.cols + i), s3 = *(const f32x4*)(sacc + 6 * a.cols + i);
        float* o = out + i;
        o[0] = (s0[0] + s1[0]) + (s2[0] + s3[0]); o[1] = (s0[1] + s1[1]) + (s2[1] + s3[1]);
        o[2] = (s0[2] + s1[2]) + (s2[2] + s3[2]); o[3] = (s0[3] + s1[3]) + (s2[3] + s3[3]);
    }
    da = block_sum<4>(da, red);
    db = block_sum<4>(db, red);
    if (threadIdx.x == 0) { out[2 * a.cols] = da; out[2 * a.cols + 1] = db; }
    FF_LTL(4);
}

template <typename T>
FF_DEV void ln_final_body(int nblk, int cols, const float* __restrict__ partial, T* dgamma, T* dbeta, const T* alpha_a, T* out_a, const T* alpha_b,
                          T* out_b) {
    __shared__ float red[16][17];
    const int P = 2 * cols + 2;
    const int tx = threadIdx.x & 15, ty = threadIdx.x >> 4;
    const int idx = blockIdx.x * 16 + tx;
    float v[8] = {0.f, 0.f, 0.f, 0.f, 0.f, 0.f, 0.f, 0.f};
    if (idx < P) {
        int b = ty;
        for (; b + 7 * 16 < nblk; b += 8 * 16) {
#pragma unroll
            for (int u = 0; u < 8; u++) v[u] += partial[(long long)(b + 16 * u) * P + idx];
        }
        for (; b < nblk; b += 16) v[0] += partial[(long long)b * P + idx];
    }
    red[ty][tx] = ((v[0] + v[1]) + (v[2] + v[3])) + ((v[4] + v[5]) + (v[6] + v[7]));
    __syncthreads();
    if (ty == 0 && idx < P) {
        float s = 0.f;
#pragma unroll
        for (int u = 0; u < 16; u++) s += red[u][tx];
        const float v = s;
        if (idx < cols) { if (dgamma) dgamma[idx] = from_f32<T>(v); }
        else if (idx < 2 * cols) { if (dbeta) dbeta[idx - cols] = from_f32<T>(v); }
        else if (idx == 2 * cols) {
            if (out_a) { const float t = tanhf(to_f32(alpha_a[0])); out_a[0] = from_f32<T>(v * (1.f - t * t)); }
        } else if (out_b) { const float t = tanhf(to_f32(alpha_b[0])); out_b[0] = from_f32<T>(v * (1.f - t * t)); }
    }
}
template <typename T>
__global__ __launch_bounds__(256) void ln_bwd_final_kernel(int nblk, int cols, const float* __restrict__ partial, T* dgamma, T* dbeta,
                                                           const T* alpha_a, T* out_a, const T* alpha_b, T* out_b) {
    pin_args(nblk, cols, partial, dgamma, dbeta, alpha_a, out_a, alpha_b, out_b);
    ln_final_body<T>(nblk, cols, partial, dgamma, dbeta, alpha_a, out_a, alpha_b, out_b);
}
struct LnFinishTable {
    LnPending s[kLnFinishMax];
};
template <typename T>
__global__ __launch_bounds__(256) void ln_bwd_final_multi_kernel(const LnFinishTable t) {
    const LnPending& e = t.s[blockIdx.y];
    if ((int)blockIdx.x * 16 >= 2 * e.cols + 2) return;
    ln_final_body<T>(e.nblk, e.cols, e.partial, (T*)e.dgamma, (T*)e.dbeta, (const T*)e.alpha_a, (T*)e.out_a, (const T*)e.alpha_b, (T*)e.out_b);
}

struct ColReduceArgs {
    int rows, cols;
    RowMap x_map, y_map;
    int rows_per_batch, rows_per_group, n_batch;
    int add_rows_per_seg, add_div;
    int rows_per_split, nsplit, ngroups;
};

template <typename T, int VEC, int MODE>
__global__ __launch_bounds__(256) void col_reduce_kernel(const ColReduceArgs a_in, const T* __restrict__ x, const T* __restrict__ dy,
                                                         const T* __restrict__ add, const float* __restrict__ mean,
                                                         const float* __restrict__ rstd, float* __restrict__ partial) {
    const ColReduceArgs a = fetch_args(a_in);
    pin_args(x, dy, add, mean, rstd, partial);
    constexpr int NS = MODE == 1 ? 2 : 1;
    __shared__ float red[4][NS][64 * VEC];
    const int tx = threadIdx.x & 63, ty = threadIdx.x >> 6;
    const int col = (blockIdx.x * 64 + tx) * VEC;
    const int g = blockIdx.y, split = blockIdx.z;
    float acc[NS][VEC];
#pragma unroll
    for (int s = 0; s < NS; s++)
#pragma unroll
        for (int i = 0; i < VEC; i++) acc[s][i] = 0.f;
    if (col < a.cols) {
        const int n_g = a.n_batch * a.rows_per_group;
        const int i_end = min(n_g, (split + 1) * a.rows_per_split);
        for (int i = split * a.rows_per_split + ty; i < i_end; i += 4) {
            const int bi = i / a.rows_per_group, j = i - bi * a.rows_per_group;
            const int row = bi * a.rows_per_batch + g * a.rows_per_group + j;
            if (row >= a.rows) continue;
            float v[VEC];
            ld<T, VEC>(x + a.x_map.off(row) + col, v);
            if (MODE == 0) {
#pragma unroll
                for (int e = 0; e < VEC; e++) acc[0][e] += v[e];
            } else {
                if (add) {
                    float t[VEC];
                    ld<T, VEC>(add + (long long)((row % a.add_rows_per_seg) / a.add_div) * a.cols + col, t);
#pragma unroll
                    for (int e = 0; e < VEC; e++) v[e] += t[e];
                }
                float d[VEC];
                ld<T, VEC>(dy + a.y_map.off(row) + col, d);
                const float mu = mean[row], rs = rstd[row];
#pragma unroll
                for (int e = 0; e < VEC; e++) {
                    acc[0][e] += d[e] * (v[e] - mu) * rs;
                    acc[1][e] += d[e];
                }
            }
        }
    }
#pragma unroll
    for (int s = 0; s < NS; s++)
#pragma unroll
        for (int e = 0; e < VEC; e++) red[ty][s][tx * VEC + e] = acc[s][e];
    __syncthreads();
    if (ty == 0 && col < a.cols) {
#pragma unroll
        for (int s = 0; s < NS; s++)
#pragma unroll
            for (int e = 0; e < VEC; e++) {
                const float v = red[0][s][tx * VEC + e] + red[1][s][tx * VEC + e] + red[2][s][tx * VEC + e] + red[3][s][tx * VEC + e];
                partial[(((long long)split * a.ngroups + g) * NS + s) * a.cols + col + e] = v;
            }
    }
}

template <typename T>
__global__ __launch_bounds__(256) void col_reduce_final_kernel(int nsplit, int ngroups, int nslots, int cols,
                                                               const float* __restrict__ partial, T* out0, T* out1) {
    pin_args(nsplit, ngroups, nslots, cols, partial, out0, out1);
    const long long total = (long long)ngroups * nslots * cols;
    for (long long idx = (long long)blockIdx.x * 256 + threadIdx.x; idx < total; idx += (long long)gridDim.x * 256) {
        float v0 = 0.f, v1 = 0.f, v2 = 0.f, v3 = 0.f;
        int s = 0;
        for (; s + 4 <= nsplit; s += 4) {
            v0 += partial[(long long)s * total + idx];
            v1 += partial[(long long)(s + 1) * total + idx];
            v2 += partial[(long long)(s + 2) * total + idx];
            v3 += partial[(long long)(s + 3) * total + idx];
        }
        for (; s < nsplit; s++) v0 += partial[(long long)s * total + idx];
        const float v = (v0 + v1) + (v2 + v3);
        const int c = (int)(idx % cols);
        const long long gs = idx / cols;
        const int slot = (int)(gs % nslots), g = (int)(gs / nslots);
        T* out = slot == 0 ? out0 : out1;
        out[(long long)g * cols + c] = from_f32<T>(v);
    }
}

template <typename T, int VEC>
__global__ __launch_bounds__(256) void dot_partial_kernel(long long n, const T* __restrict__ a, const T* __restrict__ b,
                                                          float* __restrict__ partial) {
    pin_args(n, a, b, partial);
    __shared__ float red[4];
    float s = 0.f;
    const long long nchunk = n / VEC;
    for (long long c = (long long)blockIdx.x * 256 + threadIdx.x; c < nchunk; c += (long long)gridDim.x * 256) {
        float u[VEC], v[VEC];
        ld<T, VEC>(a + c * VEC, u);
        ld<T, VEC>(b + c * VEC, v);
#pragma unroll
        for (int i = 0; i < VEC; i++) s += u[i] * v[i];
    }
    s = block_sum<4>(s, red);
    if (threadIdx.x == 0) partial[blockIdx.x] = s;
}
template <typename T>
__global__ __launch_bounds__(256) void gate_grad_final_kernel(int nblk, const float* __restrict__ partial, const T* alpha, T* dalpha) {
    pin_args(nblk, partial, alpha, dalpha);
    __shared__ float red[4];
    float s = 0.f;
    for (int i = threadIdx.x; i < nblk; i += 256) s += partial[i];
    s = block_sum<4>(s, red);
    if (threadIdx.x == 0) {
        const float t = tanhf(to_f32(alpha[0]));
        dalpha[0] = from_f32<T>(s * (1.f - t * t));
    }
}

template <typename I> __global__ void text_time_kernel(int batch, int n, const I* __restrict__ ml, int* __restrict__ out) {
    const int b = blockIdx.x * blockDim.x + threadIdx.x;
    if (b >= batch) return;
    int acc = 0;
    for (int i = 0; i < n; i++) {
        acc += (int)ml[(long long)b * n + i];
        out[(long long)b * n + i] = acc;
    }
}

int gate_grad(int dtype, int rows, int cols, const void* a, const void* b, const void* alpha, void* dalpha, void* ws,
              size_t ws_bytes, hipStream_t st_);

static bool vec_ok(int dtype, int cols, std::initializer_list<RowMap> maps, std::initializer_list<const void*> ptrs) {
    const int n = dtype == FF_DTYPE_BF16 ? 8 : 4;
    if (cols % n) return false;
    for (const RowMap& m : maps)
        if (m.ld % n || (m.rows_per_seg > 0 && m.seg_stride % n)) return false;
    for (const void* p : ptrs)
        if (p && (uintptr_t)p % 16) return false;
    return true;
}

#define FF_DISPATCH_T_VEC(dtype, vec, ...)                 \
    do {                                                    \
        if ((dtype) == FF_DTYPE_BF16) {                     \
            typedef bf16 T;                                 \
            if (vec) { constexpr int VEC = 8; __VA_ARGS__; }       \
            else { constexpr int VEC = 1; __VA_ARGS__; }           \
        } else {                                            \
            typedef float T;                                \
            if (vec) { constexpr int VEC = 4; __VA_ARGS__; }       \
            else { constexpr int VEC = 1; __VA_ARGS__; }           \
        }                                                   \
    } while (0)

int layernorm_fwd(const LnArgs& a, const void* x, const void* add, const void* gamma, const void* beta, void* y, float* mean,
                  float* rstd, hipStream_t st_) {
    FF_CHECK(a.rows > 0 && a.cols > 0 && x, FF_ERR_SHAPE, "layernorm_fwd: bad shape rows=%d cols=%d", a.rows, a.cols);
    FF_CHECK(!a.stats_given || (mean && rstd), FF_ERR_SHAPE, "layernorm_fwd: stats_given without statistics");
    FF_CHECK(!y || (gamma && beta), FF_ERR_SHAPE, "layernorm_fwd: gamma/beta missing");
    FF_CHECK(!add || (a.add_rows_per_seg > 0 && a.add_div > 0), FF_ERR_SHAPE, "layernorm_fwd: addend needs add_rows_per_seg/add_div");
    const bool v = vec_ok(a.dtype, a.cols, {a.x_map, a.y_map}, {x, add, gamma, beta, y});
    const int grid = cdiv(a.rows, 4);
    FF_DISPATCH_T_VEC(a.dtype, v, ln_fwd_kernel<T, VEC><<<dim3(grid), dim3(256), 0, st_>>>(a, (const T*)x, (const T*)add, (const T*)gamma, (const T*)beta, (T*)y, mean, rstd));
    return check_launch("ln_fwd");
}

static void split_plan(int n_rows_in_group, int col_blocks, int ngroups, int& rows_per_split, int& nsplit) {
    int target = std::max(1, 512 / std::max(1, col_blocks * ngroups));
    nsplit = std::max(1, std::min(std::min(target, 32), cdiv(n_rows_in_group, 32)));
    rows_per_split = cdiv(n_rows_in_group, nsplit);
    nsplit = cdiv(n_rows_in_group, rows_per_split);
}

static size_t col_reduce_ws(int n_rows_in_group, int cols, int ngroups, int nslots) {
    int rps, ns;
    split_plan(n_rows_in_group, 1, ngroups, rps, ns);
    return (size_t)ns * ngroups * nslots * cols * sizeof(float);
}


static int ln_fused_blocks(int rows, int& rows_per_block) {
    rows_per_block = std::max(4, (cdiv(rows, 256) + 3) / 4 * 4);
    return cdiv(rows, rows_per_block);
}
static bool ln_fused_ok(int dtype, int cols, bool vec) {
    if (!vec) return false;
    const int n = dtype == FF_DTYPE_BF16 ? 8 : 4;
    return cdiv(cols / n, 64) <= 8 && (size_t)8 * cols * sizeof(float) <= 150 * 1024;
}
size_t layernorm_bwd_workspace(int rows, int cols) {
    int rpb;
    const size_t fused = (size_t)ln_fused_blocks(rows, rpb) * (2 * (size_t)cols + 2) * sizeof(float);
    return std::max(fused, col_reduce_ws(rows, cols, 1, 2));
}

bool layernorm_bwd_deferrable(int dtype, int cols) { return cols % (dtype == FF_DTYPE_BF16 ? 8 : 4) == 0 && ln_fused_ok(dtype, cols, true); }
int layernorm_bwd_partial_blocks(int rows) {
    int rpb;
    return ln_fused_blocks(rows, rpb);
}
size_t layernorm_bwd_partial_bytes(int rows, int cols) { return (size_t)layernorm_bwd_partial_blocks(rows) * (2 * (size_t)cols + 2) * sizeof(float); }

template <typename T, int VEC>
static int launch_ln_fused(const LnArgs& a, const void* dy, const void* x, const void* add, const void* gamma, const float* mean,
                           const float* rstd, void* dx, const void* dx_res, const LnDots& dots, void* dgamma, void* dbeta, float* partial,
                           hipStream_t st_, LnPending* pending) {
    int rpb;
    const int nblk = ln_fused_blocks(a.rows, rpb);
    const int nch = cdiv(a.cols / VEC, 64);
    const size_t lds = (size_t)8 * a.cols * sizeof(float);
#define FF_LN_LAUNCH(NCH)                                                                                                                 \
    do {                                                                                                                                  \
        if (lds > 48 * 1024) {                                                                                                            \
            static bool attr[64] = {};                                                                                                    \
            int dev = 0;                                                                                                                  \
            (void)hipGetDevice(&dev);                                                                                                     \
            if (dev < 0 || dev >= 64 || !attr[dev]) {                                                                                     \
                hipFuncSetAttribute((const void*)ln_bwd_fused_kernel<T, VEC, NCH>, hipFuncAttributeMaxDynamicSharedMemorySize, 150 * 1024); \
                if (dev >= 0 && dev < 64) attr[dev] = true;                                                                               \
            }                                                                                                                             \
        }                                                                                                                                 \
        ln_bwd_fused_kernel<T, VEC, NCH><<<dim3(nblk), dim3(256), lds, st_>>>(a, (const T*)dy, (const T*)x, (const T*)add, (const T*)gamma, \
                                                                              mean, rstd, (T*)dx, (const T*)dx_res, (const T*)dots.a,     \
                                                                              (const T*)dots.b, partial, rpb);                            \
    } while (0)
    if (nch <= 2) FF_LN_LAUNCH(2);
    else if (nch <= 4) FF_LN_LAUNCH(4);
    else FF_LN_LAUNCH(8);
#undef FF_LN_LAUNCH
    FF_TRY(check_launch("ln_bwd_fused"));
    if (pending) {
        pending->partial = partial; pending->nblk = nblk; pending->cols = a.cols; pending->dgamma = dgamma; pending->dbeta = dbeta;
        pending->alpha_a = dots.alpha_a; pending->out_a = dots.out_a; pending->alpha_b = dots.alpha_b; pending->out_b = dots.out_b;
        return FF_OK;
    }
    const int P = 2 * a.cols + 2;
    ln_bwd_final_kernel<T><<<dim3(cdiv(P, 16)), dim3(256), 0, st_>>>(nblk, a.cols, partial, (T*)dgamma, (T*)dbeta, (const T*)dots.alpha_a,
                                                                     (T*)dots.out_a, (const T*)dots.alpha_b, (T*)dots.out_b);
    return check_launch("ln_bwd_final");
}

int layernorm_bwd(const LnArgs& a, const void* dy, const void* x, const void* add, const void* gamma, const float* mean,
                  const float* rstd, void* dx, const void* dx_residual, void* dgamma, void* dbeta, void* ws, size_t ws_bytes,
                  hipStream_t st_, const LnDots* dots_in, LnPending* pending) {
    FF_CHECK(a.rows > 0 && a.cols > 0 && dy && x && gamma && mean && rstd, FF_ERR_SHAPE, "layernorm_bwd: null/shape");
    if (pending) *pending = LnPending{};
    FF_CHECK(!add || (a.add_rows_per_seg > 0 && a.add_div > 0), FF_ERR_SHAPE, "layernorm_bwd: addend needs add_rows_per_seg/add_div");
    const LnDots dots = dots_in ? *dots_in : LnDots{};
    FF_CHECK(!dots.a || dx_residual, FF_ERR_SHAPE, "layernorm_bwd: dot_a is taken against dx_residual");
    FF_CHECK(!dots.b || dx, FF_ERR_SHAPE, "layernorm_bwd: dot_b is taken against dx");
    const bool v = vec_ok(a.dtype, a.cols, {a.x_map, a.y_map, a.dx_map}, {x, add, gamma, dy, dx, dx_residual, dots.a, dots.b});
    FF_CHECK(a.dy_splits == 0 || (ln_fused_ok(a.dtype, a.cols, v) && (dgamma || dots.a || dots.b) && a.cols % 4 == 0), FF_ERR_UNSUPPORTED,
             "layernorm_bwd: summing split-K slabs needs the one-pass kernel");
    if (ln_fused_ok(a.dtype, a.cols, v) && (dgamma || dots.a || dots.b)) {
        FF_CHECK(!dgamma == !dbeta, FF_ERR_SHAPE, "layernorm_bwd: dgamma and dbeta come together");
        int rpb;
        const size_t need = (size_t)ln_fused_blocks(a.rows, rpb) * (2 * (size_t)a.cols + 2) * sizeof(float);
        FF_CHECK(ws && ws_bytes >= need, FF_ERR_WORKSPACE, "layernorm_bwd workspace: need %zu have %zu", need, ws_bytes);
        if (a.dtype == FF_DTYPE_BF16) return launch_ln_fused<bf16, 8>(a, dy, x, add, gamma, mean, rstd, dx, dx_residual, dots, dgamma, dbeta, (float*)ws, st_, pending);
        return launch_ln_fused<float, 4>(a, dy, x, add, gamma, mean, rstd, dx, dx_residual, dots, dgamma, dbeta, (float*)ws, st_, pending);
    }
    if (dots.a) FF_TRY(gate_grad(a.dtype, a.rows, a.cols, dx_residual, dots.a, dots.alpha_a, dots.out_a, ws, ws_bytes, st_));
    if (dx) {
        const int grid = cdiv(a.rows, 4);
        FF_DISPATCH_T_VEC(a.dtype, v, ln_bwd_dx_kernel<T, VEC><<<dim3(grid), dim3(256), 0, st_>>>(a, (const T*)dy, (const T*)x, (const T*)add, (const T*)gamma, mean, rstd, (T*)dx, (const T*)dx_residual));
        FF_TRY(check_launch("ln_bwd_dx"));
    }
    if (dgamma || dbeta) {
        FF_CHECK(dgamma && dbeta, FF_ERR_SHAPE, "layernorm_bwd: dgamma and dbeta come together");
        const int vecn = v ? (a.dtype == FF_DTYPE_BF16 ? 8 : 4) : 1;
        ColReduceArgs c = {};
        c.rows = a.rows; c.cols = a.cols; c.x_map = a.x_map; c.y_map = a.y_map;
        c.rows_per_batch = a.rows; c.rows_per_group = a.rows; c.n_batch = 1; c.ngroups = 1;
        c.add_rows_per_seg = a.add_rows_per_seg; c.add_div = a.add_div;
        const int col_blocks = cdiv(a.cols, 64 * vecn);
        split_plan(a.rows, col_blocks, 1, c.rows_per_split, c.nsplit);
        const size_t need = (size_t)c.nsplit * 2 * a.cols * sizeof(float);
        FF_CHECK(ws && ws_bytes >= need, FF_ERR_WORKSPACE, "layernorm_bwd workspace: need %zu have %zu", need, ws_bytes);
        FF_DISPATCH_T_VEC(a.dtype, v, col_reduce_kernel<T, VEC, 1><<<dim3(col_blocks, 1, c.nsplit), dim3(256), 0, st_>>>(c, (const T*)x, (const T*)dy, (const T*)add, mean, rstd, (float*)ws));
        FF_TRY(check_launch("ln_bwd_param_partial"));
        const int grid = std::min(cdiv(2LL * a.cols, 256), 1024);
        if (a.dtype == FF_DTYPE_BF16)
            hipLaunchKernelGGL(col_reduce_final_kernel<bf16>, dim3(grid), dim3(256), 0, st_, c.nsplit, 1, 2, a.cols, (const float*)ws, (bf16*)dgamma, (bf16*)dbeta);
        else
            hipLaunchKernelGGL(col_reduce_final_kernel<float>, dim3(grid), dim3(256), 0, st_, c.nsplit, 1, 2, a.cols, (const float*)ws, (float*)dgamma, (float*)dbeta);
        FF_TRY(check_launch("ln_bwd_param_final"));
    }
    if (dots.b) FF_TRY(gate_grad(a.dtype, a.rows, a.cols, dx, dots.b, dots.alpha_b, dots.out_b, ws, ws_bytes, st_));
    return FF_OK;
}

int layernorm_bwd_finish(int dtype, const LnPending* sets, int n, hipStream_t st_) {
    for (int i0 = 0; i0 < n; i0 += kLnFinishMax) {
        LnFinishTable t = {};
        int cnt = 0, pmax = 0;
        for (int i = i0; i < n && i < i0 + kLnFinishMax; i++)
            if (sets[i].partial) {
                t.s[cnt++] = sets[i];
                pmax = std::max(pmax, 2 * sets[i].cols + 2);
            }
        if (!cnt) continue;
        const dim3 grid(cdiv(pmax, 16), cnt);
        if (dtype == FF_DTYPE_BF16) ln_bwd_final_multi_kernel<bf16><<<grid, dim3(256), 0, st_>>>(t);
        else ln_bwd_final_multi_kernel<float><<<grid, dim3(256), 0, st_>>>(t);
        FF_TRY(check_launch("ln_bwd_final_multi"));
    }
    return FF_OK;
}

size_t rows_reduce_workspace(int rows, int cols, int rows_per_batch, int rows_per_group) {
    if (rows_per_batch <= 0 || rows_per_group <= 0) return 0;
    const int ngroups = cdiv(rows_per_batch, rows_per_group);
    const int n_batch = cdiv(rows, rows_per_batch);
    return col_reduce_ws(n_batch * rows_per_group, cols, ngroups, 1);
}

int rows_reduce(int dtype, int rows, int cols, RowMap x_map, int rows_per_batch, int rows_per_group, const void* x, void* out,
                void* ws, size_t ws_bytes, hipStream_t st_) {
    FF_CHECK(rows > 0 && cols > 0 && rows_per_batch > 0 && rows_per_group > 0 && x && out, FF_ERR_SHAPE, "rows_reduce: bad arguments");
    FF_CHECK(rows % rows_per_batch == 0 && rows_per_batch % rows_per_group == 0, FF_ERR_SHAPE,
             "rows_reduce: rows=%d rows_per_batch=%d rows_per_group=%d do not nest", rows, rows_per_batch, rows_per_group);
    const bool v = vec_ok(dtype, cols, {x_map}, {x, out});
    const int vecn = v ? (dtype == FF_DTYPE_BF16 ? 8 : 4) : 1;
    ColReduceArgs c = {};
    c.rows = rows; c.cols = cols; c.x_map = x_map; c.y_map = x_map;
    c.rows_per_batch = rows_per_batch; c.rows_per_group = rows_per_group;
    c.n_batch = rows / rows_per_batch; c.ngroups = rows_per_batch / rows_per_group;
    const int col_blocks = cdiv(cols, 64 * vecn);
    split_plan(c.n_batch * rows_per_group, col_blocks, c.ngroups, c.rows_per_split, c.nsplit);
    const size_t need = (size_t)c.nsplit * c.ngroups * cols * sizeof(float);
    FF_CHECK(ws && ws_bytes >= need, FF_ERR_WORKSPACE, "rows_reduce workspace: need %zu have %zu", need, ws_bytes);
    FF_DISPATCH_T_VEC(dtype, v, col_reduce_kernel<T, VEC, 0><<<dim3(col_blocks, c.ngroups, c.nsplit), dim3(256), 0, st_>>>(c, (const T*)x, (const T*)nullptr, (const T*)nullptr, (const float*)nullptr, (const float*)nullptr, (float*)ws));
    FF_TRY(check_launch("rows_reduce_partial"));
    const int grid = std::min(cdiv((long long)c.ngroups * cols, 256), 1024);
    if (dtype == FF_DTYPE_BF16)
        hipLaunchKernelGGL(col_reduce_final_kernel<bf16>, dim3(grid), dim3(256), 0, st_, c.nsplit, c.ngroups, 1, cols, (const float*)ws, (bf16*)out, (bf16*)nullptr);
    else
        hipLaunchKernelGGL(col_reduce_final_kernel<float>, dim3(grid), dim3(256), 0, st_, c.nsplit, c.ngroups, 1, cols, (const float*)ws, (float*)out, (float*)nullptr);
    return check_launch("rows_reduce_final");
}

__global__ __launch_bounds__(256) void zero_bytes_kernel(unsigned char* __restrict__ p, size_t n) {
    for (size_t i = (size_t)blockIdx.x * 256 + threadIdx.x; i < n; i += (size_t)gridDim.x * 256) p[i] = 0;
}

int zero_bytes(void* p, size_t bytes, hipStream_t st) {
    if (bytes == 0) return 0;
    FF_CHECK(p, FF_ERR_SHAPE, "zero_bytes: null pointer");
    const int grid = (int)std::min<size_t>(1024, (bytes + 255) / 256);
    hipLaunchKernelGGL(zero_bytes_kernel, dim3(grid), dim3(256), 0, st, (unsigned char*)p, bytes);
    return check_launch("zero_bytes");
}

static int gate_blocks(long long n) { return (int)std::max<long long>(1, std::min<long long>(512, n / 4096)); }
size_t gate_grad_workspace(int rows, int cols) { return (size_t)gate_blocks((long long)rows * cols) * sizeof(float); }

int gate_grad(int dtype, int rows, int cols, const void* a, const void* b, const void* alpha, void* dalpha, void* ws,
              size_t ws_bytes, hipStream_t st_) {
    const long long n = (long long)rows * cols;
    FF_CHECK(n > 0 && a && b && alpha && dalpha, FF_ERR_SHAPE, "gate_grad: bad arguments");
    const int nblk = gate_blocks(n);
    FF_CHECK(ws && ws_bytes >= nblk * sizeof(float), FF_ERR_WORKSPACE, "gate_grad workspace too small");
    const bool v = vec_ok(dtype, cols, {}, {a, b});
    FF_DISPATCH_T_VEC(dtype, v, dot_partial_kernel<T, VEC><<<dim3(nblk), dim3(256), 0, st_>>>(n, (const T*)a, (const T*)b, (float*)ws));
    FF_TRY(check_launch("gate_grad_partial"));
    if (dtype == FF_DTYPE_BF16)
        hipLaunchKernelGGL(gate_grad_final_kernel<bf16>, dim3(1), dim3(256), 0, st_, nblk, (const float*)ws, (const bf16*)alpha, (bf16*)dalpha);
    else
        hipLaunchKernelGGL(gate_grad_final_kernel<float>, dim3(1), dim3(256), 0, st_, nblk, (const float*)ws, (const float*)alpha, (float*)dalpha);
    return check_launch("gate_grad_final");
}

int text_time(int batch, int n_tokens, const void* ml, int elem_bytes, int* out, hipStream_t st_) {
    FF_CHECK(batch > 0 && n_tokens > 0 && ml && out, FF_ERR_SHAPE, "text_time: bad arguments");
    const int grid = cdiv(batch, 64);
    if (elem_bytes == 8) hipLaunchKernelGGL(text_time_kernel<long long>, dim3(grid), dim3(64), 0, st_, batch, n_tokens, (const long long*)ml, out);
    else if (elem_bytes == 4) hipLaunchKernelGGL(text_time_kernel<int>, dim3(grid), dim3(64), 0, st_, batch, n_tokens, (const int*)ml, out);
    else if (elem_bytes == 1) hipLaunchKernelGGL(text_time_kernel<unsigned char>, dim3(grid), dim3(64), 0, st_, batch, n_tokens, (const unsigned char*)ml, out);
    else FF_CHECK(false, FF_ERR_UNSUPPORTED, "text_time: media_locations element size %d", elem_bytes);
    return check_launch("text_time");
}

}

static ff::LnArgs to_args(const ff_ln_desc* d) {
    ff::LnArgs a;
    a.dtype = d->dtype; a.rows = d->rows; a.cols = d->cols;
    a.x_map = ff::make_rowmap(d->x_map); a.y_map = ff::make_rowmap(d->y_map); a.dx_map = ff::make_rowmap(d->dx_map);
    a.add_rows_per_seg = d->add_rows_per_seg; a.add_div = d->add_div;
    a.eps = d->eps; a.stats_given = d->stats_given;
    return a;
}
extern "C" int ff_layernorm_fwd(const ff_ln_desc* d, const void* x, const void* add, const void* gamma, const void* beta, void* y,
                                float* mean, float* rstd, ff_stream_t stream) {
    return ff::layernorm_fwd(to_args(d), x, add, gamma, beta, y, mean, rstd, (hipStream_t)stream);
}
extern "C" size_t ff_layernorm_bwd_workspace_bytes(const ff_ln_desc* d) { return ff::layernorm_bwd_workspace(d->rows, d->cols); }
extern "C" int ff_layernorm_bwd(const ff_ln_desc* d, const void* dy, const void* x, const void* add, const void* gamma,
                                const float* mean, const float* rstd, void* dx, const void* dx_residual, void* dgamma, void* dbeta,
                                void* workspace, size_t workspace_bytes, ff_stream_t stream) {
    return ff::layernorm_bwd(to_args(d), dy, x, add, gamma, mean, rstd, dx, dx_residual, dgamma, dbeta, workspace, workspace_bytes,
                             (hipStream_t)stream, nullptr);
}
extern "C" size_t ff_rows_reduce_workspace_bytes(const ff_reduce_desc* d) {
    return ff::rows_reduce_workspace(d->rows, d->cols, d->rows_per_batch, d->rows_per_group);
}
extern "C" int ff_rows_reduce(const ff_reduce_desc* d, const void* x, void* out, void* workspace, size_t workspace_bytes,
                              ff_stream_t stream) {
    return ff::rows_reduce(d->dtype, d->rows, d->cols, ff::make_rowmap(d->x_map), d->rows_per_batch, d->rows_per_group, x, out,
                           workspace, workspace_bytes, (hipStream_t)stream);
}
extern "C" size_t ff_gate_grad_workspace_bytes(int rows, int cols) { return ff::gate_grad_workspace(rows, cols); }
extern "C" int ff_gate_grad(int dtype, int rows, int cols, const void* a, const void* b, const void* alpha, void* dalpha,
                            void* workspace, size_t workspace_bytes, ff_stream_t stream) {
    return ff::gate_grad(dtype, rows, cols, a, b, alpha, dalpha, workspace, workspace_bytes, (hipStream_t)stream);
}
extern "C" int ff_text_time(int batch, int n_tokens, const void* media_locations, int elem_bytes, int* text_time, ff_stream_t stream) {
    return ff::text_time(batch, n_tokens, media_locations, elem_bytes, text_time, (hipStream_t)stream);
}

#ifdef FF_XA_TIMELINE
extern "C" int ff_debug_ln_timeline_read(unsigned long long* out, int n_blocks) {
    return (int)hipMemcpyFromSymbol(out, HIP_SYMBOL(ff::g_ln_timeline), sizeof(unsigned long long) * 8 * n_blocks);
}
#endif
```

Before: 797.6.

## Skip media input gradient in resampler backward via algebraic LN/KV weight-grad path

When no gradient is needed for the media features, the resampler backward no longer builds the full media dK/dV→dkv projection or runs the per-layer media layernorm backward. Instead it computes the normalized media x-hat once, takes weight gradients for Wk/Wv against x-hat, and folds the gamma/beta and time-embedding gradients into new batched kernels (prep, rows, cols, finish, tpe). This removes the large Mf×D gemms and the per-layer LN backward over media rows. In exchange it adds several custom reduction kernels and a more intricate gradient derivation, which has more room for numerical or correctness mistakes.

```diff
diff --git a/flamingo-mini_amd/csrc/ff_api.hip b/flamingo-mini_amd/csrc/ff_api.hip
--- a/flamingo-mini_amd/csrc/ff_api.hip
+++ b/flamingo-mini_amd/csrc/ff_api.hip
@@ -46,6 +46,7 @@
     RowMap pD, pI, pF;
     RowMap lat_bcast;
     RowMap kv_media, kv_lat;
+    RowMap kvi_media, kvi_lat;
     explicit RsDims(const ff_resampler_desc& d) {
         dt = d.dtype; Bn = d.batch; T = d.n_frames; v = d.n_tokens; D = d.dim; F = T * v; q = d.num_latents;
         H = d.heads; dh = d.dim_head; inner = H * dh; ffi = d.ff_mult * D; R = F + q; depth = d.depth;
@@ -55,6 +56,8 @@
         lat_bcast = RowMap{D, 0, q};
         kv_media = RowMap{D, (long long)R * D, F};
         kv_lat = RowMap{D, (long long)R * D, q};
+        kvi_media = RowMap{inner, (long long)R * inner, F};
+        kvi_lat = RowMap{inner, (long long)R * inner, q};
     }
     LnArgs ln_latents() const { return ln_args(dt, Mq, D, pD, pD, pD); }
     LnArgs ln_media(RowMap y) const {
@@ -63,6 +66,8 @@
         return a;
     }
     template <typename P> P* kv_latent_rows(P* kv) const { return (P*)((char*)kv + (size_t)F * D * es); }
+    template <typename P> P* kvi_latent_rows(P* kv) const { return (P*)((char*)kv + (size_t)F * inner * es); }
+    RsMediaDims media() const { return rs_media_dims(dt, Bn, T, v, R, D, inner); }
 };
 struct RsLayerSaved {
     void *x_in, *kv_in, *Qs, *K, *V, *O, *x_mid, *xn_f, *Hpre, *Aact;
@@ -112,6 +117,7 @@
     g(s.Mq, s.inner, s.D, 1); g(s.Mkv, s.inner, s.D, 2); g(s.Mq, s.D, s.inner, 1); g(s.Mq, s.ffi, s.D, 1); g(s.Mq, s.D, s.ffi, 1);
     for (int nz = 1; nz <= 4; nz++) {
         g(s.D, s.ffi, s.Mq, nz); g(s.ffi, s.D, s.Mq, nz); g(s.D, s.inner, s.Mq, nz); g(s.inner, s.D, s.Mq, nz); g(s.inner, s.D, s.Mkv, nz);
+        g(s.inner, s.D, s.Mf, nz);
     }
     g(s.Mkv, s.D, s.inner, 1);
     w = std::max(w, layernorm_bwd_workspace(s.Mf, s.D));
@@ -134,10 +140,10 @@
     c.gws = c.ws_bytes - align_up(s.attn_ws);
     c.attn_ws = c.ws ? (float*)((char*)c.ws + c.gws) : nullptr;
 }
-static void rs_take_chain(const RsDims& s, Arena& a, RsChain& c) {
+static void rs_take_chain(const RsDims& s, Arena& a, RsChain& c, bool media = false) {
     c.dxn = a.take((size_t)s.Mq * s.D * s.es);
     c.dO = a.take((size_t)s.Mq * s.inner * s.es);
-    c.dkv = a.take((size_t)s.Mkv * s.D * s.es);
+    c.dkv = media ? nullptr : a.take((size_t)s.Mkv * s.D * s.es);
     c.dln = a.take((size_t)s.Mq * s.D * s.es);
 }
 static void rs_take_layer_grads(const RsDims& s, Arena& a, RsLayerGrads& g) {
@@ -147,8 +153,9 @@
     g.dK = a.take((size_t)s.Mkv * s.inner * s.es);
     g.dV = a.take((size_t)s.Mkv * s.inner * s.es);
 }
-static void rs_take_ln_partials(const RsDims& s, Arena& a, bool deferrable, float** lnp) {
-    for (int i = 0; i < 3; i++) lnp[i] = deferrable ? a.take<float>(layernorm_bwd_partial_bytes(i == 2 ? s.Mf : s.Mq, s.D)) : nullptr;
+static void rs_take_ln_partials(const RsDims& s, Arena& a, bool deferrable, float** lnp, bool media = false) {
+    for (int i = 0; i < 3; i++)
+        lnp[i] = deferrable && !(media && i == 2) ? a.take<float>(layernorm_bwd_partial_bytes(i == 2 ? s.Mf : s.Mq, s.D)) : nullptr;
 }
 
 struct RsScratch {
@@ -157,22 +164,38 @@
     void* dx_out[kMaxDepth];
     RsLayerGrads L[kMaxDepth];
     float* lnp[3 * kMaxDepth + 1];
+    void *xhat, *G[kMaxDepth];
+    float *c2u[kMaxDepth], *colpart[kMaxDepth], *svec[kMaxDepth], *finpart[kMaxDepth], *omega, *tpe_terms, *tpe_part;
 };
-static size_t rs_scratch_layout(const RsDims& s, void* base, size_t cap, bool bwd, RsScratch& o) {
+static size_t rs_scratch_layout(const RsDims& s, void* base, size_t cap, bool bwd, RsScratch& o, bool media = false) {
     Arena a(base, cap);
     rs_take_ws(s, a, o.c);
     if (bwd) {
         o.dx0 = a.take((size_t)s.Mq * s.D * s.es);
-        rs_take_chain(s, a, o.c);
-        o.dxf = a.take((size_t)s.Mf * s.D * s.es);
+        rs_take_chain(s, a, o.c, media);
+        o.dxf = media ? nullptr : a.take((size_t)s.Mf * s.D * s.es);
         for (int l = 0; l < s.depth; l++) {
             o.dx_out[l] = a.take((size_t)s.Mq * s.D * s.es);
             rs_take_layer_grads(s, a, o.L[l]);
         }
         static const int defer_ln = dbg_switch("FF_DEFER_LN", 1);
         const bool lnd = defer_ln != 0 && layernorm_bwd_deferrable(s.dt, s.D);
-        for (int l = 0; l < s.depth; l++) rs_take_ln_partials(s, a, lnd, o.lnp + 3 * l);
+        for (int l = 0; l < s.depth; l++) rs_take_ln_partials(s, a, lnd, o.lnp + 3 * l, media);
         o.lnp[3 * s.depth] = lnd ? a.take<float>(layernorm_bwd_partial_bytes(s.Mq, s.D)) : nullptr;
+        if (media) {
+            const RsMediaDims m = s.media();
+            o.xhat = a.take((size_t)s.Mf * s.D * s.es);
+            o.omega = a.take<float>((size_t)s.depth * s.Mf * 4);
+            o.tpe_terms = a.take<float>((size_t)s.depth * s.T * s.D * 4);
+            o.tpe_part = a.take<float>(rs_media_tpe_part_bytes(m));
+            for (int l = 0; l < s.depth; l++) {
+                o.G[l] = a.take((size_t)2 * s.inner * s.D * s.es);
+                o.c2u[l] = a.take<float>((size_t)4 * s.inner * 4);
+                o.colpart[l] = a.take<float>(rs_media_colpart_bytes(m));
+                o.svec[l] = a.take<float>((size_t)(1 + s.T) * 2 * s.inner * 4);
+                o.finpart[l] = a.take<float>(rs_media_finpart_bytes(m));
+            }
+        }
     }
     return align_up(a.used);
 }
@@ -242,6 +265,14 @@
     FF_TRY(rs_ln_bwd(W, lnp[0], &ln_sets[0], s.ln_latents(), W.dxn, L.x_mid, nullptr, p[8], L.mean_f, L.rstd_f, T.dx_mid, dx_out, g[8], g[9], st));
     FF_TRY(Gemm(s.dt, s.Mq, s.inner, s.D).a(0, pD).b(1, pI).c(pI).problem(T.dx_mid, p[7], W.dO).run(W.ws, W.gws, st));
     FF_TRY(attention_bwd(rs_attn_desc(s), L.Qs, L.K, L.V, nullptr, L.O, W.dO, L.lse, T.dQs, T.dK, T.dV, W.attn_ws, s.attn_ws, st));
+    if (!dx_f) {
+        const void *dK_lat = s.kvi_latent_rows(T.dK), *dV_lat = s.kvi_latent_rows(T.dV);
+        FF_TRY(Gemm(s.dt, s.Mq, s.D, s.inner).a(0, s.kvi_lat).b(1, pD).c(pD).problem(dK_lat, p[5], W.dln).run(W.ws, W.gws, st));
+        FF_TRY(Gemm(s.dt, s.Mq, s.D, s.inner).a(0, s.kvi_lat).b(1, pD).c(pD).problem(dV_lat, p[6], W.dln, nullptr, nullptr, W.dln).run(W.ws, W.gws, st));
+        FF_TRY(Gemm(s.dt, s.Mq, s.D, s.inner).a(0, pI).b(1, pD).c(pD).scale(s.scale).problem(T.dQs, p[4], W.dln, nullptr, nullptr, W.dln).run(W.ws, W.gws, st));
+        return rs_ln_bwd(W, lnp[1], &ln_sets[1], ln_args(s.dt, s.Mq, s.D, x_map, pD, pD), W.dln, x_in, nullptr, p[2], L.mean_l, L.rstd_l, dx_in, T.dx_mid,
+                         g[2], g[3], st);
+    }
     FF_TRY(Gemm(s.dt, s.Mkv, s.D, s.inner).a(0, pI).b(1, pD).c(pD).problem(T.dK, p[5], W.dkv).run(W.ws, W.gws, st));
     FF_TRY(Gemm(s.dt, s.Mkv, s.D, s.inner).a(0, pI).b(1, pD).c(pD).problem(T.dV, p[6], W.dkv, nullptr, nullptr, W.dkv).run(W.ws, W.gws, st));
     FF_TRY(Gemm(s.dt, s.Mq, s.D, s.inner).a(0, pI).b(1, pD).c(pD).res_map(s.kv_lat).scale(s.scale)
@@ -285,10 +316,12 @@
     RsSaved S;
     RsScratch W;
     FF_CHECK(rs_saved_layout(s, (void*)saved, saved_bytes, S) <= saved_bytes, FF_ERR_WORKSPACE, "resampler_bwd: saved buffer too small");
-    FF_CHECK(rs_scratch_layout(s, scratch, scratch_bytes, true, W) <= scratch_bytes, FF_ERR_WORKSPACE, "resampler_bwd: scratch too small");
+    static const int media_sw = dbg_switch("FF_RS_MEDIA", 1);
+    const bool media = !dx_f && media_sw != 0;
+    FF_CHECK(rs_scratch_layout(s, scratch, scratch_bytes, true, W, media) <= scratch_bytes, FF_ERR_WORKSPACE, "resampler_bwd: scratch too small");
     const RowMap pD = s.pD, pI = s.pI, pF = s.pF;
     const void *latents = P[0], *tpe = P[1];
-    void* dxf = dx_f ? dx_f : W.dxf;
+    void* dxf = media ? nullptr : dx_f ? dx_f : W.dxf;
     void* const ws = W.c.ws;
     const size_t gws = W.c.gws;
 
@@ -324,6 +357,51 @@
         FF_TRY(g1.run(ws, gws, st));
         FF_TRY(go.run(ws, gws, st));
         FF_TRY(gq.run(ws, gws, st));
+    }
+    if (media) {
+        const RsMediaDims md = s.media();
+        {
+            LnArgs a = s.ln_media(pD);
+            a.stats_given = 1;
+            FF_TRY(layernorm_fwd(a, x_f, tpe, nullptr, nullptr, W.xhat, S.mean_m, S.rstd_m, st));
+        }
+        Gemm gl(s.dt, s.inner, s.D, s.Mq), gg(s.dt, s.inner, s.D, s.Mf);
+        gl.a(1, s.kvi_lat).b(1, s.kv_lat).c(pD);
+        gg.a(1, s.kvi_media).b(1, pD).c(pD);
+        RsMediaTable mt = {};
+        int nl = 0;
+        for (int l = 0; l < s.depth; l++) {
+            const void* const* p = P + FF_RESAMPLER_GLOBAL_PARAMS + FF_RESAMPLER_LAYER_PARAMS * l;
+            void* const* g = G + FF_RESAMPLER_GLOBAL_PARAMS + FF_RESAMPLER_LAYER_PARAMS * l;
+            const RsLayerSaved& L = S.L[l];
+            const RsLayerGrads& T = W.L[l];
+            void* Gv = (char*)W.G[l] + (size_t)s.inner * s.D * s.es;
+            gl.problem(s.kvi_latent_rows(T.dK), s.kv_latent_rows(L.kv_in), g[5]);
+            gl.problem(s.kvi_latent_rows(T.dV), s.kv_latent_rows(L.kv_in), g[6]);
+            gg.problem(T.dK, W.xhat, W.G[l]);
+            gg.problem(T.dV, W.xhat, Gv);
+            RsMediaLayer& m = mt.L[nl++];
+            m.Wk = p[5]; m.Wv = p[6]; m.gamma = p[0]; m.beta = p[1];
+            m.dK = T.dK; m.dV = T.dV; m.K = L.K; m.V = L.V; m.G = W.G[l];
+            m.dWk = g[5]; m.dWv = g[6]; m.dgamma = g[0]; m.dbeta = g[1];
+            m.c2u = W.c2u[l]; m.colpart = W.colpart[l]; m.svec = W.svec[l]; m.finpart = W.finpart[l];
+            m.omega = W.omega + (size_t)l * s.Mf; m.tpe_terms = W.tpe_terms + (size_t)l * s.T * s.D;
+            const bool finish = nl == kRsMediaMax || l == s.depth - 1;
+            if (gl.P.nz == kRsGroup || finish) {
+                FF_TRY(gl.run(ws, gws, st));
+                FF_TRY(gg.run(ws, gws, st));
+                gl.P.nz = gg.P.nz = 0;
+            }
+            if (finish) {
+                FF_TRY(rs_media_prep(md, mt, nl, st));
+                FF_TRY(rs_media_rows(md, mt, nl, S.rstd_m, st));
+                FF_TRY(rs_media_finish(md, mt, nl, st));
+                nl = 0;
+            }
+        }
+        FF_TRY(rows_reduce(s.dt, s.Mq, s.D, s.pD, s.q, 1, W.dx0, G[0], ws, gws, st));
+        if (s.nte > s.T) FF_TRY(zero_bytes((char*)G[1] + (size_t)s.T * s.D * s.es, (size_t)(s.nte - s.T) * s.D * s.es, st));
+        return rs_media_tpe(md, s.depth, W.xhat, W.omega, W.tpe_terms, G[1], W.tpe_part, st);
     }
     {
         Gemm gkv(s.dt, s.inner, s.D, s.Mkv);
@@ -864,7 +942,8 @@
 extern "C" size_t ff_resampler_scratch_bytes(const ff_resampler_desc* d) {
     if (ff::rs_check(d) != FF_OK) return 0;
     ff::RsScratch W;
-    return ff::rs_scratch_layout(ff::RsDims(*d), nullptr, 0, true, W);
+    const ff::RsDims s(*d);
+    return std::max(ff::rs_scratch_layout(s, nullptr, 0, true, W, false), ff::rs_scratch_layout(s, nullptr, 0, true, W, true));
 }
 extern "C" int ff_resampler_fwd(const ff_resampler_desc* d, const void* x_f, const void* const* params, void* out, void* saved,
                                 size_t saved_bytes, void* scratch, size_t scratch_bytes, ff_stream_t stream) {
diff --git a/flamingo-mini_amd/csrc/ff_internal.h b/flamingo-mini_amd/csrc/ff_internal.h
--- a/flamingo-mini_amd/csrc/ff_internal.h
+++ b/flamingo-mini_amd/csrc/ff_internal.h
@@ -99,6 +99,34 @@
 int zero_bytes(void* p, size_t bytes, hipStream_t st);
 int rows_reduce(int dtype, int rows, int cols, RowMap x_map, int rows_per_batch, int rows_per_group, const void* x,
                 void* out, void* ws, size_t ws_bytes, hipStream_t st);
+
+constexpr int kRsMediaMax = 8;
+constexpr int kRsFinRows = 32;
+struct RsMediaLayer {
+    const void *Wk, *Wv, *gamma, *beta;
+    const void *dK, *dV, *K, *V;
+    const void* G;
+    void *dWk, *dWv, *dgamma, *dbeta;
+    float* c2u;
+    float* colpart;
+    float* svec;
+    float* omega;
+    float* finpart;
+    float* tpe_terms;
+};
+struct RsMediaTable { RsMediaLayer L[kRsMediaMax]; };
+struct RsMediaDims {
+    int dtype, Bn, T, v, R, D, inner;
+    int rpb, nrc;
+};
+RsMediaDims rs_media_dims(int dtype, int batch, int frames, int tokens, int kv_rows, int dim, int inner);
+inline size_t rs_media_colpart_bytes(const RsMediaDims& d) { return (size_t)d.Bn * d.T * d.nrc * 4 * d.inner * sizeof(float); }
+inline size_t rs_media_finpart_bytes(const RsMediaDims& d) { return (size_t)((2 * d.inner + kRsFinRows - 1) / kRsFinRows) * (2 + d.T) * d.D * sizeof(float); }
+size_t rs_media_tpe_part_bytes(const RsMediaDims& d);
+int rs_media_prep(const RsMediaDims& d, const RsMediaTable& t, int nl, hipStream_t st);
+int rs_media_rows(const RsMediaDims& d, const RsMediaTable& t, int nl, const float* rstd_m, hipStream_t st);
+int rs_media_finish(const RsMediaDims& d, const RsMediaTable& t, int nl, hipStream_t st);
+int rs_media_tpe(const RsMediaDims& d, int nl, const void* xhat, const float* omega, const float* tpe_terms, void* d_tpe, float* part, hipStream_t st);
 size_t gate_grad_workspace(int rows, int cols);
 int gate_grad(int dtype, int rows, int cols, const void* a, const void* b, const void* alpha, void* dalpha, void* ws,
               size_t ws_bytes, hipStream_t st);
diff --git a/flamingo-mini_amd/csrc/ff_rowwise.hip b/flamingo-mini_amd/csrc/ff_rowwise.hip
--- a/flamingo-mini_amd/csrc/ff_rowwise.hip
+++ b/flamingo-mini_amd/csrc/ff_rowwise.hip
@@ -78,10 +78,15 @@
             const int c = lane + 64 * u;
             if (c < nchunk) {
                 float g[VEC], b[VEC], o[VEC];
-                ld<T, VEC>(gamma + c * VEC, g);
-                ld<T, VEC>(beta + c * VEC, b);
-#pragma unroll
-                for (int i = 0; i < VEC; i++) o[i] = (v[u][i] - mu) * rs * g[i] + b[i];
+                if (gamma) {
+                    ld<T, VEC>(gamma + c * VEC, g);
+                    ld<T, VEC>(beta + c * VEC, b);
+#pragma unroll
+                    for (int i = 0; i < VEC; i++) o[i] = (v[u][i] - mu) * rs * g[i] + b[i];
+                } else {
+#pragma unroll
+                    for (int i = 0; i < VEC; i++) o[i] = (v[u][i] - mu) * rs;
+                }
                 st<T, VEC>(yr + c * VEC, o);
             }
         }
@@ -135,10 +140,15 @@
 #pragma unroll
             for (int i = 0; i < VEC; i++) v[i] += t[i];
         }
-        ld<T, VEC>(gamma + c * VEC, g);
-        ld<T, VEC>(beta + c * VEC, b);
-#pragma unroll
-        for (int i = 0; i < VEC; i++) v[i] = (v[i] - mu) * rs * g[i] + b[i];
+        if (gamma) {
+            ld<T, VEC>(gamma + c * VEC, g);
+            ld<T, VEC>(beta + c * VEC, b);
+#pragma unroll
+            for (int i = 0; i < VEC; i++) v[i] = (v[i] - mu) * rs * g[i] + b[i];
+        } else {
+#pragma unroll
+            for (int i = 0; i < VEC; i++) v[i] = (v[i] - mu) * rs;
+        }
         st<T, VEC>(yr + c * VEC, v);
     }
 }
@@ -517,6 +527,317 @@
     }
 }
 
+template <typename T>
+__global__ __launch_bounds__(256) void rs_media_prep_kernel(const RsMediaDims d, const RsMediaTable t) {
+    const RsMediaLayer& L = t.L[blockIdx.y];
+    const int lane = threadIdx.x & 63, c = blockIdx.x * 4 + (threadIdx.x >> 6), C = 2 * d.inner;
+    if (c >= C) return;
+    const T* w = c < d.inner ? (const T*)L.Wk + (long long)c * d.D : (const T*)L.Wv + (long long)(c - d.inner) * d.D;
+    const T *g = (const T*)L.gamma, *b = (const T*)L.beta;
+    float sb = 0.f, sg = 0.f;
+    for (int j = lane; j < d.D; j += 64) {
+        const float wv = to_f32(w[j]);
+        sb += wv * to_f32(b[j]);
+        sg += wv * to_f32(g[j]);
+    }
+    sb = wave_sum(sb);
+    sg = wave_sum(sg);
+    if (lane == 0) {
+        L.c2u[c] = sb;
+        L.c2u[C + c] = sg / (float)d.D;
+    }
+}
+
+template <typename T, int VEC>
+__global__ __launch_bounds__(256) void rs_media_rows_kernel(const RsMediaDims d, const RsMediaTable t, const float* __restrict__ rstd) {
+    constexpr int NCH = 2, W = 64 * NCH * VEC;
+    __shared__ __attribute__((aligned(16))) float sacc[4][2][W];
+    __shared__ float sb[64];
+    const RsMediaLayer& L = t.L[blockIdx.y];
+    const int lane = threadIdx.x & 63, w = threadIdx.x >> 6;
+    const int C = 2 * d.inner, nchunk = C / VEC;
+    const int blk = blockIdx.x, rc = blk % d.nrc, bt = blk / d.nrc, tt = bt % d.T, b = bt / d.T;
+    const int n0 = rc * d.rpb, n1 = min(d.v, n0 + d.rpb);
+    const long long kv0 = (long long)b * d.R + (long long)tt * d.v;
+    const long long m0 = ((long long)b * d.T + tt) * d.v;
+    float* out = L.colpart + (long long)blk * 2 * C;
+    if (threadIdx.x < 64) sb[threadIdx.x] = 0.f;
+    __syncthreads();
+    for (int ch0 = 0; ch0 < nchunk; ch0 += 64 * NCH) {
+        float as[NCH][VEC], a1[NCH][VEC], c2[NCH][VEC];
+        const T *pd[NCH], *pk[NCH];
+        bool on[NCH];
+#pragma unroll
+        for (int i = 0; i < NCH; i++) {
+            const int col = (ch0 + lane + 64 * i) * VEC;
+            on[i] = col < C;
+            const bool isk = col < d.inner;
+            const int cc = isk ? col : col - d.inner;
+            pd[i] = (const T*)(isk ? L.dK : L.dV) + cc;
+            pk[i] = (const T*)(isk ? L.K : L.V) + cc;
+#pragma unroll
+            for (int e = 0; e < VEC; e++) {
+                as[i][e] = a1[i][e] = 0.f;
+                c2[i][e] = on[i] ? L.c2u[col + e] : 0.f;
+            }
+        }
+        for (int n = n0 + w; n < n1; n += 4) {
+            const float rs = rstd[m0 + n];
+            const long long ro = (kv0 + n) * d.inner;
+            float bs = 0.f;
+#pragma unroll
+            for (int i = 0; i < NCH; i++) {
+                if (on[i]) {
+                    float dv[VEC], kv[VEC];
+                    ld<T, VEC>(pd[i] + ro, dv);
+                    ld<T, VEC>(pk[i] + ro, kv);
+#pragma unroll
+                    for (int e = 0; e < VEC; e++) {
+                        bs += dv[e] * (kv[e] - c2[i][e]);
+                        as[i][e] += dv[e];
+                        a1[i][e] += rs * dv[e];
+                    }
+                }
+            }
+            bs = wave_sum(bs);
+            if (lane == 0) sb[n - n0] += bs;
+        }
+#pragma unroll
+        for (int i = 0; i < NCH; i++)
+#pragma unroll
+            for (int e = 0; e < VEC; e++) {
+                sacc[w][0][(lane + 64 * i) * VEC + e] = as[i][e];
+                sacc[w][1][(lane + 64 * i) * VEC + e] = a1[i][e];
+            }
+        __syncthreads();
+        for (int x = threadIdx.x; x < W; x += 256) {
+            const int col = ch0 * VEC + x;
+            if (col < C) {
+                out[col] = (sacc[0][0][x] + sacc[1][0][x]) + (sacc[2][0][x] + sacc[3][0][x]);
+                out[C + col] = (sacc[0][1][x] + sacc[1][1][x]) + (sacc[2][1][x] + sacc[3][1][x]);
+            }
+        }
+        __syncthreads();
+    }
+    if ((int)threadIdx.x < n1 - n0) L.omega[m0 + n0 + threadIdx.x] = rstd[m0 + n0 + threadIdx.x] * sb[threadIdx.x] / (float)d.D;
+}
+
+__global__ __launch_bounds__(1024) void rs_media_cols_kernel(const RsMediaDims d, const RsMediaTable t) {
+    __shared__ float red[2][16][64];
+    const RsMediaLayer& L = t.L[blockIdx.y];
+    const int tx = threadIdx.x & 63, ty = threadIdx.x >> 6;
+    const int C = 2 * d.inner, c = blockIdx.x * 64 + tx;
+    const int n = d.Bn * d.nrc;
+    float s = 0.f;
+    for (int tt = 0; tt < d.T; tt++) {
+        float u0 = 0.f, u1 = 0.f, w0 = 0.f, w1 = 0.f;
+        if (c < C) {
+            int i = ty;
+            for (; i + 16 < n; i += 32) {
+                const float* p0 = L.colpart + ((long long)((i / d.nrc) * d.T + tt) * d.nrc + i % d.nrc) * 2 * C + c;
+                const float* p1 = L.colpart + ((long long)(((i + 16) / d.nrc) * d.T + tt) * d.nrc + (i + 16) % d.nrc) * 2 * C + c;
+                u0 += p0[0]; w0 += p0[C];
+                u1 += p1[0]; w1 += p1[C];
+            }
+            if (i < n) {
+                const float* p0 = L.colpart + ((long long)((i / d.nrc) * d.T + tt) * d.nrc + i % d.nrc) * 2 * C + c;
+                u0 += p0[0]; w0 += p0[C];
+            }
+        }
+        red[0][ty][tx] = u0 + u1;
+        red[1][ty][tx] = w0 + w1;
+        __syncthreads();
+        if (ty == 0 && c < C) {
+            float u = 0.f, wsum = 0.f;
+#pragma unroll
+            for (int k = 0; k < 16; k++) { u += red[0][k][tx]; wsum += red[1][k][tx]; }
+            s += u;
+            L.svec[(long long)(1 + tt) * C + c] = wsum;
+        }
+        __syncthreads();
+    }
+    if (ty == 0 && c < C) L.svec[c] = s;
+}
+
+template <typename T, int VEC>
+__global__ __launch_bounds__(256) void rs_media_finish_kernel(const RsMediaDims d, const RsMediaTable t) {
+    constexpr int KV = 4, RC = kRsFinRows, W = 64 * VEC;
+    __shared__ float ssv[RC][KV];
+    __shared__ __attribute__((aligned(16))) float red[4][1 + KV][W];
+    const RsMediaLayer& L = t.L[blockIdx.z];
+    const int lane = threadIdx.x & 63, w = threadIdx.x >> 6;
+    const int C = 2 * d.inner, nv = 1 + d.T;
+    const int col = (blockIdx.x * 64 + lane) * VEC;
+    const bool jin = col < d.D;
+    const int c0 = blockIdx.y * RC, c1 = min(C, c0 + RC);
+    float gj[VEC], bj[VEC];
+#pragma unroll
+    for (int e = 0; e < VEC; e++) gj[e] = bj[e] = 0.f;
+    if (jin) {
+        ld<T, VEC>((const T*)L.gamma + col, gj);
+        ld<T, VEC>((const T*)L.beta + col, bj);
+    }
+    float* part = L.finpart + (long long)blockIdx.y * (1 + nv) * d.D;
+    for (int k0 = 0; k0 < nv; k0 += KV) {
+        for (int i = threadIdx.x; i < RC * KV; i += 256) {
+            const int r = i / KV, k = i % KV;
+            ssv[r][k] = c0 + r < c1 && k0 + k < nv ? L.svec[(long long)(k0 + k) * C + c0 + r] : 0.f;
+        }
+        __syncthreads();
+        float dg[VEC], acc[KV][VEC];
+#pragma unroll
+        for (int e = 0; e < VEC; e++) {
+            dg[e] = 0.f;
+#pragma unroll
+            for (int k = 0; k < KV; k++) acc[k][e] = 0.f;
+        }
+        if (jin) {
+#pragma unroll
+            for (int r = w; r < RC; r += 4) {
+                const int c = c0 + r;
+                if (c < c1) {
+                    const bool isk = c < d.inner;
+                    const long long o = (long long)(isk ? c : c - d.inner) * d.D + col;
+                    float wv[VEC];
+                    ld<T, VEC>((const T*)(isk ? L.Wk : L.Wv) + o, wv);
+#pragma unroll
+                    for (int k = 0; k < KV; k++)
+#pragma unroll
+                        for (int e = 0; e < VEC; e++) acc[k][e] += wv[e] * ssv[r][k];
+                    if (k0 == 0) {
+                        T* dW = (T*)(isk ? L.dWk : L.dWv) + o;
+                        float g[VEC], lat[VEC];
+                        ld<T, VEC>((const T*)L.G + (long long)c * d.D + col, g);
+                        ld<T, VEC>(dW, lat);
+#pragma unroll
+                        for (int e = 0; e < VEC; e++) {
+                            dg[e] += wv[e] * g[e];
+                            lat[e] += gj[e] * g[e] + ssv[r][0] * bj[e];
+                        }
+                        st<T, VEC>(dW, lat);
+                    }
+                }
+            }
+        }
+#pragma unroll
+        for (int e = 0; e < VEC; e++) {
+            red[w][0][lane * VEC + e] = dg[e];
+#pragma unroll
+            for (int k = 0; k < KV; k++) red[w][1 + k][lane * VEC + e] = acc[k][e];
+        }
+        __syncthreads();
+        for (int x = threadIdx.x; x < (1 + KV) * W; x += 256) {
+            const int slot = x / W, cc = x - slot * W, j = blockIdx.x * W + cc;
+            if (j >= d.D) continue;
+            const float v = (red[0][slot][cc] + red[1][slot][cc]) + (red[2][slot][cc] + red[3][slot][cc]);
+            if (slot == 0) {
+                if (k0 == 0) part[j] = v;
+            } else if (k0 + slot - 1 < nv) part[(long long)(k0 + slot) * d.D + j] = v;
+        }
+        __syncthreads();
+    }
+}
+template <typename T>
+__global__ __launch_bounds__(256) void rs_media_finish2_kernel(const RsMediaDims d, const RsMediaTable t, int nchunk) {
+    __shared__ float red[16][17];
+    __shared__ float redb[4];
+    const RsMediaLayer& L = t.L[blockIdx.y];
+    const int tx = threadIdx.x & 15, ty = threadIdx.x >> 4;
+    const int j = blockIdx.x * 16 + tx, C = 2 * d.inner, nv = 1 + d.T;
+    for (int slot = 0; slot < 1 + nv; slot++) {
+        float us = 0.f;
+        if (slot >= 2) {
+            const float* sv = L.svec + (long long)(slot - 1) * C;
+            for (int c = threadIdx.x; c < C; c += 256) us += L.c2u[C + c] * sv[c];
+            us = block_sum<4>(us, redb);
+        }
+        float v0 = 0.f, v1 = 0.f;
+        if (j < d.D) {
+            int ch = ty;
+            for (; ch + 16 < nchunk; ch += 32) {
+                v0 += L.finpart[((long long)ch * (1 + nv) + slot) * d.D + j];
+                v1 += L.finpart[((long long)(ch + 16) * (1 + nv) + slot) * d.D + j];
+            }
+            if (ch < nchunk) v0 += L.finpart[((long long)ch * (1 + nv) + slot) * d.D + j];
+        }
+        __syncthreads();
+        red[ty][tx] = v0 + v1;
+        __syncthreads();
+        if (ty == 0 && j < d.D) {
+            float v = 0.f;
+#pragma unroll
+            for (int u = 0; u < 16; u++) v += red[u][tx];
+            if (slot == 0) ((T*)L.dgamma)[j] = from_f32<T>(v);
+            else if (slot == 1) ((T*)L.dbeta)[j] = from_f32<T>(v);
+            else L.tpe_terms[(long long)(slot - 2) * d.D + j] = to_f32(((const T*)L.gamma)[j]) * v - us;
+        }
+    }
+}
+
+template <typename T, int VEC>
+__global__ __launch_bounds__(256) void rs_media_wsum_kernel(const ColReduceArgs a_in, const T* __restrict__ x, const float* __restrict__ omega, int nl,
+                                                            float* __restrict__ partial) {
+    const ColReduceArgs a = fetch_args(a_in);
+    pin_args(x, omega, nl, partial);
+    __shared__ float red[4][64 * VEC];
+    const int tx = threadIdx.x & 63, ty = threadIdx.x >> 6;
+    const int col = (blockIdx.x * 64 + tx) * VEC;
+    const int g = blockIdx.y, split = blockIdx.z;
+    float acc[VEC];
+#pragma unroll
+    for (int e = 0; e < VEC; e++) acc[e] = 0.f;
+    if (col < a.cols) {
+        const int n_g = a.n_batch * a.rows_per_group;
+        const int i_end = min(n_g, (split + 1) * a.rows_per_split);
+        for (int i = split * a.rows_per_split + ty; i < i_end; i += 4) {
+            const int bi = i / a.rows_per_group, j = i - bi * a.rows_per_group;
+            const int row = bi * a.rows_per_batch + g * a.rows_per_group + j;
+            if (row >= a.rows) continue;
+            float om = 0.f;
+            for (int l = 0; l < nl; l++) om += omega[(long long)l * a.rows + row];
+            float v[VEC];
+            ld<T, VEC>(x + (long long)row * a.cols + col, v);
+#pragma unroll
+            for (int e = 0; e < VEC; e++) acc[e] += om * v[e];
+        }
+    }
+#pragma unroll
+    for (int e = 0; e < VEC; e++) red[ty][tx * VEC + e] = acc[e];
+    __syncthreads();
+    if (ty == 0 && col < a.cols) {
+#pragma unroll
+        for (int e = 0; e < VEC; e++)
+            partial[((long long)split * a.ngroups + g) * a.cols + col + e] =
+                (red[0][tx * VEC + e] + red[1][tx * VEC + e]) + (red[2][tx * VEC + e] + red[3][tx * VEC + e]);
+    }
+}
+template <typename T>
+__global__ __launch_bounds__(256) void rs_media_tpe_final_kernel(int nsplit, int nl, int total, const float* __restrict__ partial,
+                                                                 const float* __restrict__ terms, T* out) {
+    pin_args(nsplit, nl, total, partial, terms, out);
+    __shared__ float red[16][17];
+    const int tx = threadIdx.x & 15, ty = threadIdx.x >> 4;
+    const int idx = blockIdx.x * 16 + tx;
+    float v0 = 0.f, v1 = 0.f;
+    if (idx < total) {
+        int s = ty;
+        for (; s + 16 < nsplit; s += 32) {
+            v0 += partial[(long long)s * total + idx];
+            v1 += partial[(long long)(s + 16) * total + idx];
+        }
+        if (s < nsplit) v0 += partial[(long long)s * total + idx];
+    }
+    red[ty][tx] = v0 + v1;
+    __syncthreads();
+    if (ty == 0 && idx < total) {
+        float b = 0.f, a = 0.f;
+#pragma unroll
+        for (int u = 0; u < 16; u++) b += red[u][tx];
+        for (int l = 0; l < nl; l++) a += terms[(long long)l * total + idx];
+        out[idx] = from_f32<T>(a - b);
+    }
+}
+
 template <typename T, int VEC>
 __global__ __launch_bounds__(256) void dot_partial_kernel(long long n, const T* __restrict__ a, const T* __restrict__ b,
                                                           float* __restrict__ partial) {
@@ -587,7 +908,7 @@
                   float* rstd, hipStream_t st_) {
     FF_CHECK(a.rows > 0 && a.cols > 0 && x, FF_ERR_SHAPE, "layernorm_fwd: bad shape rows=%d cols=%d", a.rows, a.cols);
     FF_CHECK(!a.stats_given || (mean && rstd), FF_ERR_SHAPE, "layernorm_fwd: stats_given without statistics");
-    FF_CHECK(!y || (gamma && beta), FF_ERR_SHAPE, "layernorm_fwd: gamma/beta missing");
+    FF_CHECK(!gamma == !beta, FF_ERR_SHAPE, "layernorm_fwd: gamma and beta come together (both null: y = x-hat)");
     FF_CHECK(!add || (a.add_rows_per_seg > 0 && a.add_div > 0), FF_ERR_SHAPE, "layernorm_fwd: addend needs add_rows_per_seg/add_div");
     const bool v = vec_ok(a.dtype, a.cols, {a.x_map, a.y_map}, {x, add, gamma, beta, y});
     const int grid = cdiv(a.rows, 4);
@@ -770,6 +1091,89 @@
     return check_launch("rows_reduce_final");
 }
 
+RsMediaDims rs_media_dims(int dtype, int batch, int frames, int tokens, int kv_rows, int dim, int inner) {
+    RsMediaDims d;
+    d.dtype = dtype; d.Bn = batch; d.T = frames; d.v = tokens; d.R = kv_rows; d.D = dim; d.inner = inner;
+    d.nrc = cdiv(tokens, 64);
+    d.rpb = (cdiv(tokens, d.nrc) + 3) / 4 * 4;
+    d.nrc = cdiv(tokens, d.rpb);
+    return d;
+}
+static int rs_media_table_ok(const RsMediaTable& t, int nl, const char* what) {
+    FF_CHECK(nl > 0 && nl <= kRsMediaMax, FF_ERR_SHAPE, "%s: %d layers per launch", what, nl);
+    for (int l = 0; l < nl; l++) {
+        const RsMediaLayer& L = t.L[l];
+        FF_CHECK(L.Wk && L.Wv && L.gamma && L.beta && L.dK && L.dV && L.K && L.V && L.G && L.dWk && L.dWv && L.dgamma && L.dbeta && L.c2u && L.colpart &&
+                     L.svec && L.omega && L.tpe_terms,
+                 FF_ERR_SHAPE, "%s: null pointer in layer %d", what, l);
+    }
+    return FF_OK;
+}
+int rs_media_prep(const RsMediaDims& d, const RsMediaTable& t, int nl, hipStream_t st_) {
+    FF_TRY(rs_media_table_ok(t, nl, "rs_media_prep"));
+    const dim3 grid(cdiv(2 * d.inner, 4), nl);
+    if (d.dtype == FF_DTYPE_BF16) rs_media_prep_kernel<bf16><<<grid, dim3(256), 0, st_>>>(d, t);
+    else rs_media_prep_kernel<float><<<grid, dim3(256), 0, st_>>>(d, t);
+    return check_launch("rs_media_prep");
+}
+int rs_media_rows(const RsMediaDims& d, const RsMediaTable& t, int nl, const float* rstd_m, hipStream_t st_) {
+    FF_TRY(rs_media_table_ok(t, nl, "rs_media_rows"));
+    FF_CHECK(rstd_m && d.rpb > 0 && d.rpb <= 64 && d.nrc * d.rpb >= d.v, FF_ERR_SHAPE, "rs_media_rows: bad row plan");
+    bool v = d.inner % (d.dtype == FF_DTYPE_BF16 ? 8 : 4) == 0;
+    for (int l = 0; l < nl; l++)
+        for (const void* p : {t.L[l].dK, t.L[l].dV, t.L[l].K, t.L[l].V})
+            if ((uintptr_t)p % 16) v = false;
+    const dim3 grid(d.Bn * d.T * d.nrc, nl);
+    FF_DISPATCH_T_VEC(d.dtype, v, rs_media_rows_kernel<T, VEC><<<grid, dim3(256), 0, st_>>>(d, t, rstd_m));
+    FF_TRY(check_launch("rs_media_rows"));
+    rs_media_cols_kernel<<<dim3(cdiv(2 * d.inner, 64), nl), dim3(1024), 0, st_>>>(d, t);
+    return check_launch("rs_media_cols");
+}
+int rs_media_finish(const RsMediaDims& d, const RsMediaTable& t, int nl, hipStream_t st_) {
+    FF_TRY(rs_media_table_ok(t, nl, "rs_media_finish"));
+    bool v = true;
+    for (int l = 0; l < nl; l++) {
+        const RsMediaLayer& L = t.L[l];
+        FF_CHECK(L.finpart, FF_ERR_SHAPE, "rs_media_finish: null pointer in layer %d", l);
+        v = v && vec_ok(d.dtype, d.D, {}, {L.Wk, L.Wv, L.gamma, L.beta, L.G, L.dWk, L.dWv});
+    }
+    const int vecn = v ? (d.dtype == FF_DTYPE_BF16 ? 8 : 4) : 1, nchunk = cdiv(2 * d.inner, kRsFinRows);
+    const dim3 grid(cdiv(d.D, 64 * vecn), nchunk, nl);
+    FF_DISPATCH_T_VEC(d.dtype, v, rs_media_finish_kernel<T, VEC><<<grid, dim3(256), 0, st_>>>(d, t));
+    FF_TRY(check_launch("rs_media_finish"));
+    const dim3 grid2(cdiv(d.D, 16), nl);
+    if (d.dtype == FF_DTYPE_BF16) rs_media_finish2_kernel<bf16><<<grid2, dim3(256), 0, st_>>>(d, t, nchunk);
+    else rs_media_finish2_kernel<float><<<grid2, dim3(256), 0, st_>>>(d, t, nchunk);
+    return check_launch("rs_media_finish2");
+}
+static int rs_media_tpe_splits(const RsMediaDims& d, int& rows_per_split) {
+    const int n_g = d.Bn * d.v;
+    int ns = std::max(1, std::min(cdiv(n_g, 32), 512 / std::max(1, d.T)));
+    rows_per_split = cdiv(n_g, ns);
+    return cdiv(n_g, rows_per_split);
+}
+size_t rs_media_tpe_part_bytes(const RsMediaDims& d) {
+    int rps;
+    return (size_t)rs_media_tpe_splits(d, rps) * d.T * d.D * sizeof(float);
+}
+int rs_media_tpe(const RsMediaDims& d, int nl, const void* xhat, const float* omega, const float* tpe_terms, void* d_tpe, float* part, hipStream_t st_) {
+    FF_CHECK(nl > 0 && xhat && omega && tpe_terms && d_tpe && part, FF_ERR_SHAPE, "rs_media_tpe: bad arguments");
+    const int F = d.T * d.v, rows = d.Bn * F;
+    const bool v = vec_ok(d.dtype, d.D, {}, {xhat});
+    const int vecn = v ? (d.dtype == FF_DTYPE_BF16 ? 8 : 4) : 1;
+    ColReduceArgs c = {};
+    c.rows = rows; c.cols = d.D; c.x_map = plain_rows(d.D); c.y_map = c.x_map;
+    c.rows_per_batch = F; c.rows_per_group = d.v; c.n_batch = d.Bn; c.ngroups = d.T;
+    c.nsplit = rs_media_tpe_splits(d, c.rows_per_split);
+    const int col_blocks = cdiv(d.D, 64 * vecn);
+    FF_DISPATCH_T_VEC(d.dtype, v, rs_media_wsum_kernel<T, VEC><<<dim3(col_blocks, c.ngroups, c.nsplit), dim3(256), 0, st_>>>(c, (const T*)xhat, omega, nl, part));
+    FF_TRY(check_launch("rs_media_wsum"));
+    const int total = d.T * d.D;
+    if (d.dtype == FF_DTYPE_BF16) rs_media_tpe_final_kernel<bf16><<<dim3(cdiv(total, 16)), dim3(256), 0, st_>>>(c.nsplit, nl, total, part, tpe_terms, (bf16*)d_tpe);
+    else rs_media_tpe_final_kernel<float><<<dim3(cdiv(total, 16)), dim3(256), 0, st_>>>(c.nsplit, nl, total, part, tpe_terms, (float*)d_tpe);
+    return check_launch("rs_media_tpe_final");
+}
+
 __global__ __launch_bounds__(256) void zero_bytes_kernel(unsigned char* __restrict__ p, size_t n) {
     for (size_t i = (size_t)blockIdx.x * 256 + threadIdx.x; i < n; i += (size_t)gridDim.x * 256) p[i] = 0;
 }
```

After: 802.3 (median of 6 runs). No clear change (+0.6%).
